# Dhia-naouali/dinov3-jax

Hardware: AMD Instinct MI355X
Metric: images/sec (whole node) ViT-L/16 DINOv3 pretrain 224px (higher is better)
Workload: dtype bf16; 1 GPU; model=vit_large, global_batch=64, img_size=224, local_crops=8, parallelism=dp1

## Files before the change

dinov3_amd/ops/csrc/bindings.hip:

```cpp

#include <torch/extension.h>
#include <ATen/hip/HIPContext.h>
#include <hip/hip_runtime.h>
#include <hip/hip_bf16.h>

#include <vector>

#define CHECK_INPUT(x) \
  TORCH_CHECK(x.is_cuda() && x.is_contiguous(), #x " must be a contiguous HIP tensor")

template <typename T>
void launch_layernorm_fwd(const T*, const T*, const T*, T*, float*, float*, long, int,
                          float, hipStream_t);
template <typename T>
void launch_layernorm_bwd(const T*, const T*, const T*, const float*, const float*, T*,
                          float*, float*, long, int, hipStream_t);
template <typename T>
void launch_rmsnorm_fwd(const T*, const T*, T*, float*, long, int, float, hipStream_t);
template <typename T>
void launch_rmsnorm_bwd(const T*, const T*, const T*, const float*, T*, float*, long, int,
                        hipStream_t);
template <typename T>
void launch_l2norm_fwd(const T*, T*, float*, long, int, float, hipStream_t);
template <typename T>
void launch_l2norm_bwd(const T*, const T*, const float*, T*, long, int, float, hipStream_t);
template <typename T>
void launch_bias_gelu_fwd(const T*, const T*, T*, long, int, hipStream_t);
template <typename T>
void launch_bias_gelu_bwd(const T*, const T*, const T*, T*, float*, long, int, hipStream_t);
template <typename T>
void launch_ls_axpy_fwd(const T*, const T*, const T*, T*, long, int, hipStream_t);
template <typename T>
void launch_ls_axpy_bwd(const T*, const T*, const T*, T*, float*, long, int, hipStream_t);
template <typename T>
void launch_ls_axpy_bias_fwd(const T*, const T*, const T*, const T*, T*, long, int,
                             hipStream_t);
template <typename T>
void launch_ls_axpy_bias_bwd(const T*, const T*, const T*, const T*, T*, float*, float*,
                             long, int, hipStream_t);
template <typename T>
void launch_ls_scatter_add(T*, const long*, const T*, const T*, const T*, const float*,
                           long, int, hipStream_t);
template <typename T>
void launch_ls_scatter_bwd(const T*, const long*, const T*, const T*, const T*,
                           const float*, T*, float*, float*, long, int, hipStream_t);
template <typename T>
void launch_row_gather(const T*, const long*, T*, long, int, hipStream_t);
template <typename T>
void launch_row_scatter_add(T*, const long*, const T*, const float*, long, int,
                            hipStream_t);
template <typename T>
void launch_row_gather_scaled(const T*, const long*, const float*, T*, long, int,
                              hipStream_t);
template <typename T>
void launch_swiglu_fwd(const T*, T*, long, int, hipStream_t);
template <typename T>
void launch_swiglu_bwd(const T*, const T*, T*, long, int, hipStream_t);
template <typename T>
void launch_rope_fwd(const T*, const float*, const float*, T*, long, int, int, int,
                     hipStream_t);
void launch_dino_ce_fwd(const __hip_bfloat16*, const float*, float*, float*, float*, int,
                        int, int, long, float, bool, hipStream_t);
void launch_dino_ce_bwd(const __hip_bfloat16*, const float*, const float*, const float*,
                        const float*, __hip_bfloat16*, int, int, int, long, float, bool,
                        hipStream_t);
void launch_ibot_ce_fwd(const __hip_bfloat16*, const float*, const float*, float*, float*,
                        float*, int, long, float, hipStream_t);
void launch_ibot_ce_bwd(const __hip_bfloat16*, const float*, const float*, const float*,
                        const float*, const float*, __hip_bfloat16*, int, long, float,
                        hipStream_t);
void launch_sinkhorn_exp(const __hip_bfloat16*, float*, float*, long, float, hipStream_t);
void launch_sinkhorn_fact_colsum(const __hip_bfloat16*, const float*, float*, int, long,
                                 float, hipStream_t);
void launch_sinkhorn_fact_rowsum(const __hip_bfloat16*, const float*, float*, int, long,
                                 float, hipStream_t);
void launch_ibot_ce_fact_fwd(const __hip_bfloat16*, const __hip_bfloat16*, const float*,
                             const float*, const float*, float*, float*, float*, int,
                             long, float, float, hipStream_t);
void launch_ibot_ce_fact_bwd(const __hip_bfloat16*, const __hip_bfloat16*, const float*,
                             const float*, const float*, const float*, const float*,
                             const float*, __hip_bfloat16*, int, long, float, float,
                             hipStream_t);
void launch_dino_ce_fact_fwd(const __hip_bfloat16*, const __hip_bfloat16*, const float*,
                             const float*, float*, float*, float*, int, int, int, long,
                             float, float, bool, hipStream_t);
void launch_dino_ce_fact_bwd(const __hip_bfloat16*, const __hip_bfloat16*, const float*,
                             const float*, const float*, const float*, const float*,
                             __hip_bfloat16*, int, int, int, long, float, float, bool,
                             hipStream_t);
void launch_sinkhorn_colsum(const float*, float*, int, long, const float*, hipStream_t);
void launch_sinkhorn_div_row(float*, const float*, int, long, float, const float*, bool,
                             hipStream_t);
void launch_fmha_rope_fwd(const __hip_bfloat16*, const float*, const float*,
                          __hip_bfloat16*, float*, int, int, int, int, int, float,
                          hipStream_t);
void launch_fmha_rope_bwd_pre(const __hip_bfloat16*, const __hip_bfloat16*, float*, int,
                              int, int, int, hipStream_t);
void launch_fmha_rope_bwd_dq(const __hip_bfloat16*, const __hip_bfloat16*, const float*,
                             const float*, const float*, const float*, __hip_bfloat16*,
                             int, int, int, int, int, float, hipStream_t);
void launch_fmha_rope_bwd_dkv(const __hip_bfloat16*, const __hip_bfloat16*, const float*,
                              const float*, const float*, const float*, __hip_bfloat16*,
                              int, int, int, int, int, float, hipStream_t);
void launch_patch_embed_fwd(const __hip_bfloat16*, const __hip_bfloat16*,
                            const __hip_bfloat16*, __hip_bfloat16*, int, int, int, int,
                            int, int, hipStream_t);
void launch_probe_mfma(const __hip_bfloat16*, const __hip_bfloat16*, float*, hipStream_t);
void launch_fmha_fwd(const __hip_bfloat16*, const __hip_bfloat16*, const __hip_bfloat16*,
                     __hip_bfloat16*, float*, int, int, int, float, hipStream_t);
void launch_fmha_bwd_pre(const __hip_bfloat16*, const __hip_bfloat16*, float*, long, int,
                         hipStream_t);
void launch_fmha_bwd_dq(const __hip_bfloat16*, const __hip_bfloat16*, const __hip_bfloat16*,
                        const __hip_bfloat16*, const float*, const float*, __hip_bfloat16*,
                        int, int, int, float, hipStream_t);
void launch_fmha_bwd_dkv(const __hip_bfloat16*, const __hip_bfloat16*,
                         const __hip_bfloat16*, const __hip_bfloat16*, const float*,
                         const float*, __hip_bfloat16*, __hip_bfloat16*, int, int, int,
                         float, hipStream_t);
template <typename T>
void launch_multi_tensor_ema(T* const*, const T* const*, const long*, const int*,
                             const long*, int, float, hipStream_t);
template <typename T>
void launch_multi_tensor_adamw(T* const*, const T* const*, float* const*, float* const*,
                               float* const*, const long*, const int*, const long*, int,
                               float, float, float, float, float, float, float, float,
                               bool, hipStream_t);
template <typename T>
void launch_multi_tensor_l2norm_sq(const T* const*, const long*, const int*, const long*,
                                   int, float*, hipStream_t);
template <typename T, typename GT>
void launch_multi_tensor_adamw_planned(T* const*, const GT* const*, float* const*,
                                       float* const*, float* const*, const long*,
                                       const int*, const long*, int, const float*,
                                       const float*, const float*, const int*,
                                       const float*, float, float, float, float, float,
                                       float, float, float, bool, hipStream_t);
template <typename T>
void launch_multi_tensor_l2norm_planned(const T* const*, const long*, const int*,
                                        const long*, int, const int*, float*,
                                        hipStream_t);

namespace {

hipStream_t current_stream() { return at::hip::getCurrentHIPStream().stream(); }

#define DISPATCH_FLOAT_BF16(TYPE, NAME, ...)                                   \
  [&] {                                                                        \
    if (TYPE == at::ScalarType::Float) {                                       \
      using scalar_t = float;                                                  \
      return __VA_ARGS__();                                                    \
    } else if (TYPE == at::ScalarType::BFloat16) {                             \
      using scalar_t = __hip_bfloat16;                                         \
      return __VA_ARGS__();                                                    \
    } else {                                                                   \
      TORCH_CHECK(false, NAME ": unsupported dtype ", TYPE);                   \
    }                                                                          \
  }()


std::vector<torch::Tensor> layernorm_fwd(torch::Tensor x, torch::Tensor w, torch::Tensor b,
                                         double eps) {
  CHECK_INPUT(x);
  const int D = x.size(-1);
  const long rows = x.numel() / D;
  auto y = torch::empty_like(x);
  auto mean = torch::empty({rows}, x.options().dtype(torch::kFloat));
  auto rstd = torch::empty({rows}, x.options().dtype(torch::kFloat));
  DISPATCH_FLOAT_BF16(x.scalar_type(), "layernorm_fwd", [&] {
    launch_layernorm_fwd<scalar_t>(
        (const scalar_t*)x.data_ptr(), (const scalar_t*)w.data_ptr(),
        (const scalar_t*)b.data_ptr(), (scalar_t*)y.data_ptr(),
        mean.data_ptr<float>(), rstd.data_ptr<float>(), rows, D, (float)eps,
        current_stream());
  });
  return {y, mean, rstd};
}

std::vector<torch::Tensor> layernorm_bwd(torch::Tensor dy, torch::Tensor x, torch::Tensor w,
                                         torch::Tensor mean, torch::Tensor rstd) {
  CHECK_INPUT(dy);
  CHECK_INPUT(x);
  const int D = x.size(-1);
  const long rows = x.numel() / D;
  auto dx = torch::empty_like(x);
  auto dw = torch::zeros({32, D}, x.options().dtype(torch::kFloat));
  auto db = torch::zeros({32, D}, x.options().dtype(torch::kFloat));
  DISPATCH_FLOAT_BF16(x.scalar_type(), "layernorm_bwd", [&] {
    launch_layernorm_bwd<scalar_t>(
        (const scalar_t*)dy.data_ptr(), (const scalar_t*)x.data_ptr(),
        (const scalar_t*)w.data_ptr(), mean.data_ptr<float>(), rstd.data_ptr<float>(),
        (scalar_t*)dx.data_ptr(), dw.data_ptr<float>(), db.data_ptr<float>(), rows, D,
        current_stream());
  });
  return {dx, dw.sum(0).to(x.scalar_type()), db.sum(0).to(x.scalar_type())};
}

std::vector<torch::Tensor> rmsnorm_fwd(torch::Tensor x, torch::Tensor w, double eps) {
  CHECK_INPUT(x);
  const int D = x.size(-1);
  const long rows = x.numel() / D;
  auto y = torch::empty_like(x);
  auto rstd = torch::empty({rows}, x.options().dtype(torch::kFloat));
  DISPATCH_FLOAT_BF16(x.scalar_type(), "rmsnorm_fwd", [&] {
    launch_rmsnorm_fwd<scalar_t>((const scalar_t*)x.data_ptr(), (const scalar_t*)w.data_ptr(),
                                 (scalar_t*)y.data_ptr(), rstd.data_ptr<float>(), rows, D,
                                 (float)eps, current_stream());
  });
  return {y, rstd};
}

std::vector<torch::Tensor> rmsnorm_bwd(torch::Tensor dy, torch::Tensor x, torch::Tensor w,
                                       torch::Tensor rstd) {
  CHECK_INPUT(dy);
  const int D = x.size(-1);
  const long rows = x.numel() / D;
  auto dx = torch::empty_like(x);
  auto dw = torch::zeros({D}, x.options().dtype(torch::kFloat));
  DISPATCH_FLOAT_BF16(x.scalar_type(), "rmsnorm_bwd", [&] {
    launch_rmsnorm_bwd<scalar_t>((const scalar_t*)dy.data_ptr(), (const scalar_t*)x.data_ptr(),
                                 (const scalar_t*)w.data_ptr(), rstd.data_ptr<float>(),
                                 (scalar_t*)dx.data_ptr(), dw.data_ptr<float>(), rows, D,
                                 current_stream());
  });
  return {dx, dw.to(x.scalar_type())};
}

std::vector<torch::Tensor> l2norm_fwd(torch::Tensor x, double eps) {
  CHECK_INPUT(x);
  const int D = x.size(-1);
  const long rows = x.numel() / D;
  auto y = torch::empty_like(x);
  auto s = torch::empty({rows}, x.options().dtype(torch::kFloat));
  DISPATCH_FLOAT_BF16(x.scalar_type(), "l2norm_fwd", [&] {
    launch_l2norm_fwd<scalar_t>((const scalar_t*)x.data_ptr(), (scalar_t*)y.data_ptr(),
                                s.data_ptr<float>(), rows, D, (float)eps, current_stream());
  });
  return {y, s};
}

torch::Tensor l2norm_bwd(torch::Tensor dy, torch::Tensor y, torch::Tensor s, double eps) {
  CHECK_INPUT(dy);
  const int D = y.size(-1);
  const long rows = y.numel() / D;
  auto dx = torch::empty_like(y);
  DISPATCH_FLOAT_BF16(y.scalar_type(), "l2norm_bwd", [&] {
    launch_l2norm_bwd<scalar_t>((const scalar_t*)dy.data_ptr(), (const scalar_t*)y.data_ptr(),
                                s.data_ptr<float>(), (scalar_t*)dx.data_ptr(), rows, D,
                                (float)eps, current_stream());
  });
  return dx;
}


torch::Tensor bias_gelu_fwd(torch::Tensor x, torch::Tensor bias) {
  CHECK_INPUT(x);
  const int H = x.size(-1);
  TORCH_CHECK(H % 8 == 0, "bias_gelu: H must be a multiple of 8");
  const long rows = x.numel() / H;
  auto y = torch::empty_like(x);
  DISPATCH_FLOAT_BF16(x.scalar_type(), "bias_gelu_fwd", [&] {
    launch_bias_gelu_fwd<scalar_t>((const scalar_t*)x.data_ptr(),
                                   (const scalar_t*)bias.data_ptr(), (scalar_t*)y.data_ptr(),
                                   rows, H, current_stream());
  });
  return y;
}

std::vector<torch::Tensor> bias_gelu_bwd(torch::Tensor dy, torch::Tensor x,
                                         torch::Tensor bias) {
  CHECK_INPUT(dy);
  const int H = x.size(-1);
  const long rows = x.numel() / H;
  auto dx = torch::empty_like(x);
  auto dbias = torch::zeros({32, H}, x.options().dtype(torch::kFloat));
  DISPATCH_FLOAT_BF16(x.scalar_type(), "bias_gelu_bwd", [&] {
    launch_bias_gelu_bwd<scalar_t>((const scalar_t*)dy.data_ptr(),
                                   (const scalar_t*)x.data_ptr(),
                                   (const scalar_t*)bias.data_ptr(), (scalar_t*)dx.data_ptr(),
                                   dbias.data_ptr<float>(), rows, H, current_stream());
  });
  return {dx, dbias.sum(0).to(x.scalar_type())};
}

torch::Tensor ls_axpy_fwd(torch::Tensor x, torch::Tensor res, torch::Tensor gamma) {
  CHECK_INPUT(x);
  CHECK_INPUT(res);
  const int D = x.size(-1);
  TORCH_CHECK(D % 8 == 0, "ls_axpy: D must be a multiple of 8");
  const long rows = x.numel() / D;
  auto out = torch::empty_like(x);
  DISPATCH_FLOAT_BF16(x.scalar_type(), "ls_axpy_fwd", [&] {
    launch_ls_axpy_fwd<scalar_t>((const scalar_t*)x.data_ptr(),
                                 (const scalar_t*)res.data_ptr(),
                                 (const scalar_t*)gamma.data_ptr(),
                                 (scalar_t*)out.data_ptr(), rows, D, current_stream());
  });
  return out;
}

torch::Tensor ls_axpy_bias_fwd(torch::Tensor x, torch::Tensor res, torch::Tensor gamma,
                               torch::Tensor bias) {
  CHECK_INPUT(x);
  CHECK_INPUT(res);
  const int D = x.size(-1);
  TORCH_CHECK(D % 8 == 0, "ls_axpy_bias: D must be a multiple of 8");
  const long rows = x.numel() / D;
  auto out = torch::empty_like(x);
  DISPATCH_FLOAT_BF16(x.scalar_type(), "ls_axpy_bias_fwd", [&] {
    launch_ls_axpy_bias_fwd<scalar_t>(
        (const scalar_t*)x.data_ptr(), (const scalar_t*)res.data_ptr(),
        (const scalar_t*)gamma.data_ptr(), (const scalar_t*)bias.data_ptr(),
        (scalar_t*)out.data_ptr(), rows, D, current_stream());
  });
  return out;
}

std::vector<torch::Tensor> ls_axpy_bwd(torch::Tensor dout, torch::Tensor res,
                                       torch::Tensor gamma) {
  CHECK_INPUT(dout);
  const int D = dout.size(-1);
  const long rows = dout.numel() / D;
  auto dres = torch::empty_like(dout);
  auto dgamma = torch::zeros({32, D}, dout.options().dtype(torch::kFloat));
  DISPATCH_FLOAT_BF16(dout.scalar_type(), "ls_axpy_bwd", [&] {
    launch_ls_axpy_bwd<scalar_t>((const scalar_t*)dout.data_ptr(),
                                 (const scalar_t*)res.data_ptr(),
                                 (const scalar_t*)gamma.data_ptr(),
                                 (scalar_t*)dres.data_ptr(), dgamma.data_ptr<float>(),
                                 rows, D, current_stream());
  });
  return {dres, dgamma.sum(0).to(dout.scalar_type())};
}

std::vector<torch::Tensor> ls_axpy_bias_bwd(torch::Tensor dout, torch::Tensor res,
                                            torch::Tensor gamma, torch::Tensor bias) {
  CHECK_INPUT(dout);
  const int D = dout.size(-1);
  const long rows = dout.numel() / D;
  auto dres = torch::empty_like(dout);
  auto fopt = dout.options().dtype(torch::kFloat);
  auto dgamma = torch::zeros({32, D}, fopt);
  auto dbias = torch::zeros({32, D}, fopt);
  DISPATCH_FLOAT_BF16(dout.scalar_type(), "ls_axpy_bias_bwd", [&] {
    launch_ls_axpy_bias_bwd<scalar_t>(
        (const scalar_t*)dout.data_ptr(), (const scalar_t*)res.data_ptr(),
        (const scalar_t*)gamma.data_ptr(), (const scalar_t*)bias.data_ptr(),
        (scalar_t*)dres.data_ptr(), dgamma.data_ptr<float>(), dbias.data_ptr<float>(),
        rows, D, current_stream());
  });
  return {dres, dgamma.sum(0).to(dout.scalar_type()), dbias.sum(0).to(dout.scalar_type())};
}

torch::Tensor row_gather(torch::Tensor src, torch::Tensor idx) {
  CHECK_INPUT(src);
  const int D = src.size(-1);
  TORCH_CHECK(D % 8 == 0, "row ops need D % 8 == 0");
  const long M = idx.numel();
  auto out = torch::empty({M, D}, src.options());
  DISPATCH_FLOAT_BF16(src.scalar_type(), "row_gather", [&] {
    launch_row_gather<scalar_t>((const scalar_t*)src.data_ptr(), idx.data_ptr<long>(),
                                (scalar_t*)out.data_ptr(), M, D, current_stream());
  });
  return out;
}

void row_scatter_add_(torch::Tensor dst, torch::Tensor idx, torch::Tensor src,
                      torch::Tensor scale) {
  CHECK_INPUT(dst);
  CHECK_INPUT(src);
  const int D = dst.size(-1);
  const long M = idx.numel();
  const float* sp = (scale.defined() && scale.numel() > 0) ? scale.data_ptr<float>() : nullptr;
  DISPATCH_FLOAT_BF16(dst.scalar_type(), "row_scatter_add", [&] {
    launch_row_scatter_add<scalar_t>((scalar_t*)dst.data_ptr(), idx.data_ptr<long>(),
                                     (const scalar_t*)src.data_ptr(), sp, M, D,
                                     current_stream());
  });
}

torch::Tensor row_gather_scaled(torch::Tensor src, torch::Tensor idx, torch::Tensor scale) {
  CHECK_INPUT(src);
  const int D = src.size(-1);
  const long M = idx.numel();
  auto out = torch::empty({M, D}, src.options());
  const float* sp = (scale.defined() && scale.numel() > 0) ? scale.data_ptr<float>() : nullptr;
  DISPATCH_FLOAT_BF16(src.scalar_type(), "row_gather_scaled", [&] {
    launch_row_gather_scaled<scalar_t>((const scalar_t*)src.data_ptr(),
                                       idx.data_ptr<long>(), sp, (scalar_t*)out.data_ptr(),
                                       M, D, current_stream());
  });
  return out;
}

void ls_scatter_add_(torch::Tensor dst, torch::Tensor idx, torch::Tensor src,
                     torch::Tensor gamma, torch::Tensor bias, torch::Tensor scale) {
  CHECK_INPUT(dst);
  CHECK_INPUT(src);
  const int D = dst.size(-1);
  TORCH_CHECK(D % 8 == 0, "ls_scatter: D must be a multiple of 8");
  const long M = idx.numel();
  DISPATCH_FLOAT_BF16(dst.scalar_type(), "ls_scatter_add_", [&] {
    launch_ls_scatter_add<scalar_t>(
        (scalar_t*)dst.data_ptr(), idx.data_ptr<long>(), (const scalar_t*)src.data_ptr(),
        gamma.defined() ? (const scalar_t*)gamma.data_ptr() : nullptr,
        bias.defined() ? (const scalar_t*)bias.data_ptr() : nullptr,
        scale.defined() && scale.numel() > 0 ? scale.data_ptr<float>() : nullptr, M, D,
        current_stream());
  });
}

std::vector<torch::Tensor> ls_scatter_bwd(torch::Tensor dy, torch::Tensor idx,
                                          torch::Tensor src, torch::Tensor gamma,
                                          torch::Tensor bias, torch::Tensor scale) {
  CHECK_INPUT(dy);
  CHECK_INPUT(src);
  const int D = dy.size(-1);
  const long M = idx.numel();
  auto dres = torch::empty_like(src);
  auto fopt = dy.options().dtype(torch::kFloat);
  auto dgamma = gamma.defined() ? torch::zeros({32, D}, fopt) : torch::Tensor();
  auto dbias = bias.defined() ? torch::zeros({32, D}, fopt) : torch::Tensor();
  DISPATCH_FLOAT_BF16(dy.scalar_type(), "ls_scatter_bwd", [&] {
    launch_ls_scatter_bwd<scalar_t>(
        (const scalar_t*)dy.data_ptr(), idx.data_ptr<long>(),
        (const scalar_t*)src.data_ptr(),
        gamma.defined() ? (const scalar_t*)gamma.data_ptr() : nullptr,
        bias.defined() ? (const scalar_t*)bias.data_ptr() : nullptr,
        scale.defined() && scale.numel() > 0 ? scale.data_ptr<float>() : nullptr,
        (scalar_t*)dres.data_ptr(),
        dgamma.defined() ? dgamma.data_ptr<float>() : nullptr,
        dbias.defined() ? dbias.data_ptr<float>() : nullptr, M, D, current_stream());
  });
  return {dres, dgamma.defined() ? dgamma.sum(0).to(dy.scalar_type()) : dgamma,
          dbias.defined() ? dbias.sum(0).to(dy.scalar_type()) : dbias};
}

torch::Tensor swiglu_fwd(torch::Tensor x12) {
  CHECK_INPUT(x12);
  const int H2 = x12.size(-1);
  const int H = H2 / 2;
  const long rows = x12.numel() / H2;
  auto sizes = x12.sizes().vec();
  sizes.back() = H;
  auto y = torch::empty(sizes, x12.options());
  DISPATCH_FLOAT_BF16(x12.scalar_type(), "swiglu_fwd", [&] {
    launch_swiglu_fwd<scalar_t>((const scalar_t*)x12.data_ptr(), (scalar_t*)y.data_ptr(),
                                rows, H, current_stream());
  });
  return y;
}

torch::Tensor swiglu_bwd(torch::Tensor dy, torch::Tensor x12) {
  CHECK_INPUT(dy);
  const int H2 = x12.size(-1);
  const int H = H2 / 2;
  const long rows = x12.numel() / H2;
  auto dx12 = torch::empty_like(x12);
  DISPATCH_FLOAT_BF16(x12.scalar_type(), "swiglu_bwd", [&] {
    launch_swiglu_bwd<scalar_t>((const scalar_t*)dy.data_ptr(),
                                (const scalar_t*)x12.data_ptr(), (scalar_t*)dx12.data_ptr(),
                                rows, H, current_stream());
  });
  return dx12;
}

torch::Tensor rope_fwd(torch::Tensor x, torch::Tensor sin_t, torch::Tensor cos_t,
                       int64_t prefix) {
  CHECK_INPUT(x);
  TORCH_CHECK(x.dim() == 4, "rope_fwd expects [B, H, N, hd]");
  TORCH_CHECK(sin_t.scalar_type() == at::ScalarType::Float, "rope tables must be fp32");
  const long BH = x.size(0) * x.size(1);
  const int N = x.size(2);
  const int hd = x.size(3);
  const int P = N - (int)prefix;
  TORCH_CHECK(sin_t.size(0) == P && sin_t.size(1) == hd, "rope table shape mismatch");
  auto y = torch::empty_like(x);
  DISPATCH_FLOAT_BF16(x.scalar_type(), "rope_fwd", [&] {
    launch_rope_fwd<scalar_t>((const scalar_t*)x.data_ptr(), sin_t.data_ptr<float>(),
                              cos_t.data_ptr<float>(), (scalar_t*)y.data_ptr(), BH, N, P, hd,
                              current_stream());
  });
  return y;
}


std::vector<torch::Tensor> dino_ce_fwd(torch::Tensor x, torch::Tensor t, double temp,
                                       bool ignore_diag) {
  CHECK_INPUT(x);
  CHECK_INPUT(t);
  TORCH_CHECK(x.dim() == 3 && t.dim() == 3, "dino_ce expects [S,B,K] and [T,B,K]");
  TORCH_CHECK(x.scalar_type() == at::ScalarType::BFloat16);
  TORCH_CHECK(t.scalar_type() == at::ScalarType::Float);
  const int S = x.size(0), B = x.size(1);
  const int T = t.size(0);
  const long K = x.size(2);
  auto lse = torch::empty({S * B}, x.options().dtype(torch::kFloat));
  auto st = torch::empty({S * B}, x.options().dtype(torch::kFloat));
  auto loss = torch::zeros({}, x.options().dtype(torch::kFloat));
  launch_dino_ce_fwd((const __hip_bfloat16*)x.data_ptr(), t.data_ptr<float>(),
                     lse.data_ptr<float>(), st.data_ptr<float>(), loss.data_ptr<float>(),
                     S, T, B, K, (float)(1.0 / temp), ignore_diag, current_stream());
  return {loss, lse, st};
}

torch::Tensor dino_ce_bwd(torch::Tensor g, torch::Tensor x, torch::Tensor t,
                          torch::Tensor lse, torch::Tensor st, double temp,
                          bool ignore_diag) {
  const int S = x.size(0), B = x.size(1);
  const int T = t.size(0);
  const long K = x.size(2);
  auto dx = torch::empty_like(x);
  launch_dino_ce_bwd((const __hip_bfloat16*)x.data_ptr(), t.data_ptr<float>(),
                     lse.data_ptr<float>(), st.data_ptr<float>(), g.data_ptr<float>(),
                     (__hip_bfloat16*)dx.data_ptr(), S, T, B, K, (float)(1.0 / temp),
                     ignore_diag, current_stream());
  return dx;
}

std::vector<torch::Tensor> ibot_ce_fwd(torch::Tensor x, torch::Tensor t, torch::Tensor w,
                                       double temp) {
  CHECK_INPUT(x);
  CHECK_INPUT(t);
  const int M = x.size(0);
  const long K = x.size(1);
  auto lse = torch::empty({M}, x.options().dtype(torch::kFloat));
  auto st = torch::empty({M}, x.options().dtype(torch::kFloat));
  auto loss = torch::zeros({}, x.options().dtype(torch::kFloat));
  launch_ibot_ce_fwd((const __hip_bfloat16*)x.data_ptr(), t.data_ptr<float>(),
                     w.data_ptr<float>(), lse.data_ptr<float>(), st.data_ptr<float>(),
                     loss.data_ptr<float>(), M, K, (float)(1.0 / temp), current_stream());
  return {loss, lse, st};
}

torch::Tensor ibot_ce_bwd(torch::Tensor g, torch::Tensor x, torch::Tensor t,
                          torch::Tensor w, torch::Tensor lse, torch::Tensor st,
                          double temp) {
  const int M = x.size(0);
  const long K = x.size(1);
  auto dx = torch::empty_like(x);
  launch_ibot_ce_bwd((const __hip_bfloat16*)x.data_ptr(), t.data_ptr<float>(),
                     w.data_ptr<float>(), lse.data_ptr<float>(), st.data_ptr<float>(),
                     g.data_ptr<float>(), (__hip_bfloat16*)dx.data_ptr(), M, K,
                     (float)(1.0 / temp), current_stream());
  return dx;
}

torch::Tensor sinkhorn_fact_colsum(torch::Tensor x, torch::Tensor u, double temp) {
  CHECK_INPUT(x);
  const int M = x.size(0);
  const long K = x.size(1);
  auto A = torch::empty({K}, x.options().dtype(torch::kFloat));
  const float* up = (u.defined() && u.numel() > 0) ? u.data_ptr<float>() : nullptr;
  launch_sinkhorn_fact_colsum((const __hip_bfloat16*)x.data_ptr(), up,
                              A.data_ptr<float>(), M, K, (float)(1.0 / temp),
                              current_stream());
  return A;
}

torch::Tensor sinkhorn_fact_rowsum(torch::Tensor x, torch::Tensor v, double temp) {
  CHECK_INPUT(x);
  const int M = x.size(0);
  const long K = x.size(1);
  auto u = torch::empty({M}, x.options().dtype(torch::kFloat));
  launch_sinkhorn_fact_rowsum((const __hip_bfloat16*)x.data_ptr(), v.data_ptr<float>(),
                              u.data_ptr<float>(), M, K, (float)(1.0 / temp),
                              current_stream());
  return u;
}

std::vector<torch::Tensor> ibot_ce_fact_fwd(torch::Tensor x, torch::Tensor xt,
                                            torch::Tensor u, torch::Tensor v,
                                            torch::Tensor w, double temp, double tt) {
  CHECK_INPUT(x);
  CHECK_INPUT(xt);
  const int M = x.size(0);
  const long K = x.size(1);
  auto lse = torch::empty({M}, x.options().dtype(torch::kFloat));
  auto st = torch::empty({M}, x.options().dtype(torch::kFloat));
  auto loss = torch::zeros({}, x.options().dtype(torch::kFloat));
  launch_ibot_ce_fact_fwd((const __hip_bfloat16*)x.data_ptr(),
                          (const __hip_bfloat16*)xt.data_ptr(), u.data_ptr<float>(),
                          v.data_ptr<float>(), w.data_ptr<float>(), lse.data_ptr<float>(),
                          st.data_ptr<float>(), loss.data_ptr<float>(), M, K,
                          (float)(1.0 / temp), (float)(1.0 / tt), current_stream());
  return {loss, lse, st};
}

torch::Tensor ibot_ce_fact_bwd(torch::Tensor g, torch::Tensor x, torch::Tensor xt,
                               torch::Tensor u, torch::Tensor v, torch::Tensor w,
                               torch::Tensor lse, torch::Tensor st, double temp,
                               double tt) {
  const int M = x.size(0);
  const long K = x.size(1);
  auto dx = torch::empty_like(x);
  launch_ibot_ce_fact_bwd((const __hip_bfloat16*)x.data_ptr(),
                          (const __hip_bfloat16*)xt.data_ptr(), u.data_ptr<float>(),
                          v.data_ptr<float>(), w.data_ptr<float>(), lse.data_ptr<float>(),
                          st.data_ptr<float>(), g.data_ptr<float>(),
                          (__hip_bfloat16*)dx.data_ptr(), M, K, (float)(1.0 / temp),
                          (float)(1.0 / tt), current_stream());
  return dx;
}

std::vector<torch::Tensor> dino_ce_fact_fwd(torch::Tensor x, torch::Tensor xt,
                                            torch::Tensor u, torch::Tensor v, double temp,
                                            double tt, bool ignore_diag) {
  CHECK_INPUT(x);
  CHECK_INPUT(xt);
  const int S = x.size(0), B = x.size(1);
  const int T = xt.size(0);
  const long K = x.size(2);
  auto lse = torch::empty({S * B}, x.options().dtype(torch::kFloat));
  auto st = torch::empty({S * B}, x.options().dtype(torch::kFloat));
  auto loss = torch::zeros({}, x.options().dtype(torch::kFloat));
  launch_dino_ce_fact_fwd((const __hip_bfloat16*)x.data_ptr(),
                          (const __hip_bfloat16*)xt.data_ptr(), u.data_ptr<float>(),
                          v.data_ptr<float>(), lse.data_ptr<float>(), st.data_ptr<float>(),
                          loss.data_ptr<float>(), S, T, B, K, (float)(1.0 / temp),
                          (float)(1.0 / tt), ignore_diag, current_stream());
  return {loss, lse, st};
}

torch::Tensor dino_ce_fact_bwd(torch::Tensor g, torch::Tensor x, torch::Tensor xt,
                               torch::Tensor u, torch::Tensor v, torch::Tensor lse,
                               torch::Tensor st, double temp, double tt,
                               bool ignore_diag) {
  const int S = x.size(0), B = x.size(1);
  const int T = xt.size(0);
  const long K = x.size(2);
  auto dx = torch::empty_like(x);
  launch_dino_ce_fact_bwd((const __hip_bfloat16*)x.data_ptr(),
                          (const __hip_bfloat16*)xt.data_ptr(), u.data_ptr<float>(),
                          v.data_ptr<float>(), lse.data_ptr<float>(), st.data_ptr<float>(),
                          g.data_ptr<float>(), (__hip_bfloat16*)dx.data_ptr(), S, T, B, K,
                          (float)(1.0 / temp), (float)(1.0 / tt), ignore_diag,
                          current_stream());
  return dx;
}

std::vector<torch::Tensor> sinkhorn_exp(torch::Tensor x, double temp) {
  CHECK_INPUT(x);
  auto Q = torch::empty(x.sizes(), x.options().dtype(torch::kFloat));
  auto total = torch::zeros({}, x.options().dtype(torch::kFloat));
  launch_sinkhorn_exp((const __hip_bfloat16*)x.data_ptr(), Q.data_ptr<float>(),
                      total.data_ptr<float>(), x.numel(), (float)(1.0 / temp),
                      current_stream());
  return {Q, total};
}

torch::Tensor sinkhorn_colsum(torch::Tensor Q, torch::Tensor divisor) {
  const int M = Q.size(0);
  const long K = Q.size(1);
  auto out = torch::empty({K}, Q.options());
  launch_sinkhorn_colsum(Q.data_ptr<float>(), out.data_ptr<float>(), M, K,
                         divisor.data_ptr<float>(), current_stream());
  return out;
}

void sinkhorn_div_row(torch::Tensor Q, torch::Tensor col, double k_div, torch::Tensor B,
                      bool scale_back) {
  const int M = Q.size(0);
  const long K = Q.size(1);
  launch_sinkhorn_div_row(Q.data_ptr<float>(), col.data_ptr<float>(), M, K, (float)k_div,
                          B.data_ptr<float>(), scale_back, current_stream());
}


torch::Tensor probe_mfma(torch::Tensor A, torch::Tensor B) {
  CHECK_INPUT(A);
  CHECK_INPUT(B);
  TORCH_CHECK(A.scalar_type() == at::ScalarType::BFloat16);
  auto C = torch::empty({32, 32}, A.options().dtype(torch::kFloat));
  launch_probe_mfma((const __hip_bfloat16*)A.data_ptr(), (const __hip_bfloat16*)B.data_ptr(),
                    C.data_ptr<float>(), current_stream());
  return C;
}

std::vector<torch::Tensor> fmha_fwd(torch::Tensor q, torch::Tensor k, torch::Tensor v) {
  CHECK_INPUT(q);
  CHECK_INPUT(k);
  CHECK_INPUT(v);
  TORCH_CHECK(q.scalar_type() == at::ScalarType::BFloat16, "fmha: bf16 only");
  TORCH_CHECK(q.dim() == 4, "fmha expects [B, H, N, hd]");
  const int B = q.size(0), H = q.size(1), N = q.size(2), HD = q.size(3);
  TORCH_CHECK(HD == 64 || HD == 128, "fmha: head_dim must be 64 or 128, got ", HD);
  auto o = torch::empty_like(q);
  auto lse = torch::empty({B, H, N}, q.options().dtype(torch::kFloat));
  const float scale = 1.0f / std::sqrt((float)HD);
  launch_fmha_fwd((const __hip_bfloat16*)q.data_ptr(), (const __hip_bfloat16*)k.data_ptr(),
                  (const __hip_bfloat16*)v.data_ptr(), (__hip_bfloat16*)o.data_ptr(),
                  lse.data_ptr<float>(), B * H, N, HD, scale, current_stream());
  return {o, lse};
}

std::vector<torch::Tensor> fmha_bwd(torch::Tensor dout, torch::Tensor q, torch::Tensor k,
                                    torch::Tensor v, torch::Tensor o, torch::Tensor lse) {
  CHECK_INPUT(dout);
  const int B = q.size(0), H = q.size(1), N = q.size(2), HD = q.size(3);
  const float scale = 1.0f / std::sqrt((float)HD);
  auto D = torch::empty({B, H, N}, q.options().dtype(torch::kFloat));
  auto dq = torch::empty_like(q);
  auto dk = torch::empty_like(k);
  auto dv = torch::empty_like(v);
  auto stream = current_stream();
  launch_fmha_bwd_pre((const __hip_bfloat16*)dout.data_ptr(),
                      (const __hip_bfloat16*)o.data_ptr(), D.data_ptr<float>(),
                      (long)B * H * N, HD, stream);
  launch_fmha_bwd_dq((const __hip_bfloat16*)q.data_ptr(), (const __hip_bfloat16*)k.data_ptr(),
                     (const __hip_bfloat16*)v.data_ptr(),
                     (const __hip_bfloat16*)dout.data_ptr(), lse.data_ptr<float>(),
                     D.data_ptr<float>(), (__hip_bfloat16*)dq.data_ptr(), B * H, N, HD,
                     scale, stream);
  launch_fmha_bwd_dkv((const __hip_bfloat16*)q.data_ptr(), (const __hip_bfloat16*)k.data_ptr(),
                      (const __hip_bfloat16*)v.data_ptr(),
                      (const __hip_bfloat16*)dout.data_ptr(), lse.data_ptr<float>(),
                      D.data_ptr<float>(), (__hip_bfloat16*)dk.data_ptr(),
                      (__hip_bfloat16*)dv.data_ptr(), B * H, N, HD, scale, stream);
  return {dq, dk, dv};
}


torch::Tensor patch_embed_fwd(torch::Tensor x, torch::Tensor w, torch::Tensor bias,
                              int64_t patch) {
  CHECK_INPUT(x);
  CHECK_INPUT(w);
  TORCH_CHECK(x.dim() == 4 && x.scalar_type() == at::ScalarType::BFloat16);
  const int B = x.size(0), C = x.size(1), H = x.size(2), W = x.size(3);
  const int D = w.size(0);
  TORCH_CHECK(C == 3, "patch_embed_fwd kernel supports C=3 (any patch size)");
  TORCH_CHECK(H % patch == 0 && W % patch == 0, "H/W must be multiples of patch");
  const long rows = (long)B * (H / patch) * (W / patch);
  auto out = torch::empty({(long)B, rows / B, (long)D}, x.options());
  launch_patch_embed_fwd((const __hip_bfloat16*)x.data_ptr(),
                         (const __hip_bfloat16*)w.data_ptr(),
                         (const __hip_bfloat16*)bias.data_ptr(),
                         (__hip_bfloat16*)out.data_ptr(), B, C, H, W, (int)patch, D,
                         current_stream());
  return out;
}


std::vector<torch::Tensor> fmha_rope_fwd_out(torch::Tensor qkv, torch::Tensor sin_t,
                                             torch::Tensor cos_t, int64_t prefix,
                                             torch::Tensor out_o) {
  CHECK_INPUT(qkv);
  TORCH_CHECK(qkv.dim() == 5 && qkv.size(2) == 3, "qkv must be [B, N, 3, H, hd]");
  TORCH_CHECK(qkv.scalar_type() == at::ScalarType::BFloat16);
  const int B = qkv.size(0), N = qkv.size(1), H = qkv.size(3), HD = qkv.size(4);
  TORCH_CHECK(HD == 64 || HD == 128, "head_dim must be 64 or 128");
  const bool has_rope = sin_t.defined() && sin_t.numel() > 0;
  const int P = has_rope ? (int)sin_t.size(0) : N - (int)prefix;
  if (has_rope) {
    TORCH_CHECK(sin_t.scalar_type() == at::ScalarType::Float && sin_t.is_contiguous());
    TORCH_CHECK(P == N - prefix, "rope table rows must equal N - prefix");
  }
  torch::Tensor o = out_o.defined() && out_o.numel() > 0 ? out_o
                                                        : torch::empty({B, N, H, HD}, qkv.options());
  TORCH_CHECK(o.is_contiguous() && o.numel() == (long)B * N * H * HD);
  auto lse = torch::empty({B, H, N}, qkv.options().dtype(torch::kFloat));
  const float scale = 1.0f / std::sqrt((float)HD);
  launch_fmha_rope_fwd((const __hip_bfloat16*)qkv.data_ptr(),
                       has_rope ? sin_t.data_ptr<float>() : nullptr,
                       has_rope ? cos_t.data_ptr<float>() : nullptr,
                       (__hip_bfloat16*)o.data_ptr(), lse.data_ptr<float>(), B, H, N, P,
                       HD, scale, current_stream());
  return {o, lse};
}

torch::Tensor fmha_rope_bwd_out(torch::Tensor dout, torch::Tensor qkv, torch::Tensor o,
                                torch::Tensor lse, torch::Tensor sin_t,
                                torch::Tensor cos_t, int64_t prefix,
                                torch::Tensor out_dqkv) {
  CHECK_INPUT(dout);
  const int B = qkv.size(0), N = qkv.size(1), H = qkv.size(3), HD = qkv.size(4);
  const bool has_rope = sin_t.defined() && sin_t.numel() > 0;
  const int P = N - (int)prefix;
  const float scale = 1.0f / std::sqrt((float)HD);
  auto D = torch::empty({B, H, N}, qkv.options().dtype(torch::kFloat));
  torch::Tensor dqkv = out_dqkv.defined() && out_dqkv.numel() > 0 ? out_dqkv
                                                                  : torch::empty_like(qkv);
  auto stream = current_stream();
  launch_fmha_rope_bwd_pre((const __hip_bfloat16*)dout.data_ptr(),
                           (const __hip_bfloat16*)o.data_ptr(), D.data_ptr<float>(), B, H,
                           N, HD, stream);
  launch_fmha_rope_bwd_dq((const __hip_bfloat16*)qkv.data_ptr(),
                          (const __hip_bfloat16*)dout.data_ptr(),
                          has_rope ? sin_t.data_ptr<float>() : nullptr,
                          has_rope ? cos_t.data_ptr<float>() : nullptr,
                          lse.data_ptr<float>(), D.data_ptr<float>(),
                          (__hip_bfloat16*)dqkv.data_ptr(), B, H, N, P, HD, scale, stream);
  launch_fmha_rope_bwd_dkv((const __hip_bfloat16*)qkv.data_ptr(),
                           (const __hip_bfloat16*)dout.data_ptr(),
                           has_rope ? sin_t.data_ptr<float>() : nullptr,
                           has_rope ? cos_t.data_ptr<float>() : nullptr,
                           lse.data_ptr<float>(), D.data_ptr<float>(),
                           (__hip_bfloat16*)dqkv.data_ptr(), B, H, N, P, HD, scale,
                           stream);
  return dqkv;
}



void multi_tensor_ema_planned(torch::Tensor ptrs, torch::Tensor sizes, torch::Tensor ct,
                              torch::Tensor co, int64_t n_tensors, double m,
                              bool is_bf16) {
  const int n_chunks = (int)ct.numel();
  long* pp = ptrs.data_ptr<long>();
  if (is_bf16) {
    launch_multi_tensor_ema<__hip_bfloat16>(
        (__hip_bfloat16* const*)pp, (const __hip_bfloat16* const*)(pp + n_tensors),
        sizes.data_ptr<long>(), ct.data_ptr<int>(), co.data_ptr<long>(), n_chunks,
        (float)m, current_stream());
  } else {
    launch_multi_tensor_ema<float>(
        (float* const*)pp, (const float* const*)(pp + n_tensors), sizes.data_ptr<long>(),
        ct.data_ptr<int>(), co.data_ptr<long>(), n_chunks, (float)m, current_stream());
  }
}

void multi_tensor_adamw_planned(torch::Tensor ptrs, torch::Tensor sizes, torch::Tensor ct,
                                torch::Tensor co, int64_t n_tensors, torch::Tensor lr_mult,
                                torch::Tensor wd_mult, torch::Tensor is_last,
                                torch::Tensor sub_id, torch::Tensor clip, double lr,
                                double last_lr, double wd, double beta1, double beta2,
                                double eps, double bc1, double bc2, bool has_master,
                                bool is_bf16, bool grad_is_f32) {
  const int n_chunks = (int)ct.numel();
  long* pp = ptrs.data_ptr<long>();
  const long n = n_tensors;
  if (is_bf16 && grad_is_f32) {
    launch_multi_tensor_adamw_planned<__hip_bfloat16, float>(
        (__hip_bfloat16* const*)pp, (const float* const*)(pp + n),
        (float* const*)(pp + 2 * n), (float* const*)(pp + 3 * n),
        has_master ? (float* const*)(pp + 4 * n) : nullptr, sizes.data_ptr<long>(),
        ct.data_ptr<int>(), co.data_ptr<long>(), n_chunks, lr_mult.data_ptr<float>(),
        wd_mult.data_ptr<float>(), is_last.data_ptr<float>(), sub_id.data_ptr<int>(),
        clip.data_ptr<float>(), (float)lr, (float)last_lr, (float)wd, (float)beta1,
        (float)beta2, (float)eps, (float)bc1, (float)bc2, has_master, current_stream());
  } else if (is_bf16) {
    launch_multi_tensor_adamw_planned<__hip_bfloat16, __hip_bfloat16>(
        (__hip_bfloat16* const*)pp, (const __hip_bfloat16* const*)(pp + n),
        (float* const*)(pp + 2 * n), (float* const*)(pp + 3 * n),
        has_master ? (float* const*)(pp + 4 * n) : nullptr, sizes.data_ptr<long>(),
        ct.data_ptr<int>(), co.data_ptr<long>(), n_chunks, lr_mult.data_ptr<float>(),
        wd_mult.data_ptr<float>(), is_last.data_ptr<float>(), sub_id.data_ptr<int>(),
        clip.data_ptr<float>(), (float)lr, (float)last_lr, (float)wd, (float)beta1,
        (float)beta2, (float)eps, (float)bc1, (float)bc2, has_master, current_stream());
  } else {
    launch_multi_tensor_adamw_planned<float, float>(
        (float* const*)pp, (const float* const*)(pp + n), (float* const*)(pp + 2 * n),
        (float* const*)(pp + 3 * n), has_master ? (float* const*)(pp + 4 * n) : nullptr,
        sizes.data_ptr<long>(), ct.data_ptr<int>(), co.data_ptr<long>(), n_chunks,
        lr_mult.data_ptr<float>(), wd_mult.data_ptr<float>(), is_last.data_ptr<float>(),
        sub_id.data_ptr<int>(), clip.data_ptr<float>(), (float)lr, (float)last_lr,
        (float)wd, (float)beta1, (float)beta2, (float)eps, (float)bc1, (float)bc2,
        has_master, current_stream());
  }
}

torch::Tensor multi_tensor_l2norm_planned(torch::Tensor ptrs, torch::Tensor sizes,
                                          torch::Tensor ct, torch::Tensor co,
                                          torch::Tensor sub_id, int64_t n_submodels,
                                          bool is_bf16) {
  const int n_chunks = (int)ct.numel();
  auto out = torch::zeros({n_submodels}, torch::dtype(torch::kFloat).device(ptrs.device()));
  long* pp = ptrs.data_ptr<long>();
  if (is_bf16) {
    launch_multi_tensor_l2norm_planned<__hip_bfloat16>(
        (const __hip_bfloat16* const*)pp, sizes.data_ptr<long>(), ct.data_ptr<int>(),
        co.data_ptr<long>(), n_chunks, sub_id.data_ptr<int>(), out.data_ptr<float>(),
        current_stream());
  } else {
    launch_multi_tensor_l2norm_planned<float>(
        (const float* const*)pp, sizes.data_ptr<long>(), ct.data_ptr<int>(),
        co.data_ptr<long>(), n_chunks, sub_id.data_ptr<int>(), out.data_ptr<float>(),
        current_stream());
  }
  return out;
}


struct MTTables {
  torch::Tensor device_buf;
  long* sizes;
  int* chunk_tensor;
  long* chunk_offset;
  long* ptr_arrays;
  int n_chunks;
  int n_tensors;
};

constexpr long kMTChunk = 65536;

MTTables build_tables(const std::vector<std::vector<torch::Tensor>>& lists,
                      torch::Device device) {
  const int n_tensors = (int)lists[0].size();
  const int n_lists = (int)lists.size();
  std::vector<long> sizes(n_tensors);
  std::vector<int> chunk_tensor;
  std::vector<long> chunk_offset;
  for (int t = 0; t < n_tensors; ++t) {
    sizes[t] = lists[0][t].numel();
    for (long off = 0; off < sizes[t]; off += kMTChunk) {
      chunk_tensor.push_back(t);
      chunk_offset.push_back(off);
    }
  }
  const int n_chunks = (int)chunk_tensor.size();
  const long total = n_tensors + n_chunks + n_chunks + (long)n_lists * n_tensors;
  auto host = torch::empty({total}, torch::dtype(torch::kLong).pinned_memory(true));
  long* hp = host.data_ptr<long>();
  long* p_sizes = hp;
  long* p_ct = hp + n_tensors;
  long* p_co = p_ct + n_chunks;
  long* p_ptr = p_co + n_chunks;
  for (int t = 0; t < n_tensors; ++t) p_sizes[t] = sizes[t];
  for (int c = 0; c < n_chunks; ++c) {
    p_ct[c] = chunk_tensor[c];
    p_co[c] = chunk_offset[c];
  }
  for (int l = 0; l < n_lists; ++l)
    for (int t = 0; t < n_tensors; ++t)
      p_ptr[(long)l * n_tensors + t] = (long)(uintptr_t)lists[l][t].data_ptr();
  auto dev = host.to(device, true);
  MTTables out;
  out.device_buf = dev;
  long* dp = dev.data_ptr<long>();
  out.sizes = dp;
  out.chunk_tensor = nullptr;
  out.chunk_offset = dp + n_tensors + n_chunks;
  out.ptr_arrays = dp + n_tensors + 2 * (long)n_chunks;
  out.n_chunks = n_chunks;
  out.n_tensors = n_tensors;
  return out;
}

torch::Tensor build_chunk_tensor_i32(const std::vector<long>& sizes, torch::Device device,
                                     int* n_chunks_out) {
  std::vector<int> ct;
  for (int t = 0; t < (int)sizes.size(); ++t)
    for (long off = 0; off < sizes[t]; off += kMTChunk) ct.push_back(t);
  *n_chunks_out = (int)ct.size();
  auto host = torch::from_blob(ct.data(), {(long)ct.size()}, torch::kInt).clone();
  return host.to(device);
}

void multi_tensor_ema(std::vector<torch::Tensor> t_list, std::vector<torch::Tensor> s_list,
                      double m) {
  TORCH_CHECK(!t_list.empty() && t_list.size() == s_list.size());
  auto device = t_list[0].device();
  auto tables = build_tables({t_list, s_list}, device);
  std::vector<long> sizes(tables.n_tensors);
  for (int t = 0; t < tables.n_tensors; ++t) sizes[t] = t_list[t].numel();
  int n_chunks;
  auto ct32 = build_chunk_tensor_i32(sizes, device, &n_chunks);
  auto stream = current_stream();
  DISPATCH_FLOAT_BF16(t_list[0].scalar_type(), "multi_tensor_ema", [&] {
    launch_multi_tensor_ema<scalar_t>(
        (scalar_t* const*)(tables.ptr_arrays),
        (const scalar_t* const*)(tables.ptr_arrays + tables.n_tensors),
        tables.sizes, ct32.data_ptr<int>(), tables.chunk_offset, n_chunks, (float)m, stream);
  });
}

void multi_tensor_adamw(std::vector<torch::Tensor> p, std::vector<torch::Tensor> g,
                        std::vector<torch::Tensor> m, std::vector<torch::Tensor> v,
                        std::vector<torch::Tensor> w, double lr, double beta1, double beta2,
                        double eps, double weight_decay, double bc1, double bc2,
                        double grad_scale) {
  TORCH_CHECK(!p.empty());
  const bool has_master = !w.empty();
  auto device = p[0].device();
  std::vector<std::vector<torch::Tensor>> lists = {p, g, m, v};
  if (has_master) lists.push_back(w);
  auto tables = build_tables(lists, device);
  std::vector<long> sizes(tables.n_tensors);
  for (int t = 0; t < tables.n_tensors; ++t) sizes[t] = p[t].numel();
  int n_chunks;
  auto ct32 = build_chunk_tensor_i32(sizes, device, &n_chunks);
  auto stream = current_stream();
  const int nt = tables.n_tensors;
  DISPATCH_FLOAT_BF16(p[0].scalar_type(), "multi_tensor_adamw", [&] {
    launch_multi_tensor_adamw<scalar_t>(
        (scalar_t* const*)(tables.ptr_arrays),
        (const scalar_t* const*)(tables.ptr_arrays + nt),
        (float* const*)(tables.ptr_arrays + 2L * nt),
        (float* const*)(tables.ptr_arrays + 3L * nt),
        has_master ? (float* const*)(tables.ptr_arrays + 4L * nt) : nullptr,
        tables.sizes, ct32.data_ptr<int>(), tables.chunk_offset, n_chunks, (float)lr,
        (float)beta1, (float)beta2, (float)eps, (float)weight_decay, (float)bc1, (float)bc2,
        (float)grad_scale, has_master, stream);
  });
}

torch::Tensor multi_tensor_l2norm_sq(std::vector<torch::Tensor> g) {
  TORCH_CHECK(!g.empty());
  auto device = g[0].device();
  auto tables = build_tables({g}, device);
  std::vector<long> sizes(tables.n_tensors);
  for (int t = 0; t < tables.n_tensors; ++t) sizes[t] = g[t].numel();
  int n_chunks;
  auto ct32 = build_chunk_tensor_i32(sizes, device, &n_chunks);
  auto out = torch::zeros({}, torch::dtype(torch::kFloat).device(device));
  DISPATCH_FLOAT_BF16(g[0].scalar_type(), "multi_tensor_l2norm_sq", [&] {
    launch_multi_tensor_l2norm_sq<scalar_t>(
        (const scalar_t* const*)(tables.ptr_arrays), tables.sizes, ct32.data_ptr<int>(),
        tables.chunk_offset, n_chunks, out.data_ptr<float>(), current_stream());
  });
  return out;
}

}

std::vector<torch::Tensor> blaslt_gemm_bias_gelu_fwd(torch::Tensor x, torch::Tensor w,
                                                     torch::Tensor bias);
std::vector<torch::Tensor> blaslt_gemm_dgelu_bgrad(torch::Tensor dy, torch::Tensor w2,
                                                   torch::Tensor pre);
torch::Tensor blaslt_gemm_bias(torch::Tensor x, torch::Tensor w, torch::Tensor bias);
int64_t blaslt_probe_epilogue(int64_t epi, int64_t aux_type, int64_t bias_type,
                              int64_t m, int64_t n, int64_t k);

PYBIND11_MODULE(TORCH_EXTENSION_NAME, mod) {
  mod.def("blaslt_gemm_bias_gelu_fwd", &blaslt_gemm_bias_gelu_fwd);
  mod.def("blaslt_gemm_dgelu_bgrad", &blaslt_gemm_dgelu_bgrad);
  mod.def("blaslt_gemm_bias", &blaslt_gemm_bias);
  mod.def("blaslt_probe_epilogue", &blaslt_probe_epilogue);
  mod.def("layernorm_fwd", &layernorm_fwd);
  mod.def("layernorm_bwd", &layernorm_bwd);
  mod.def("rmsnorm_fwd", &rmsnorm_fwd);
  mod.def("rmsnorm_bwd", &rmsnorm_bwd);
  mod.def("l2norm_fwd", &l2norm_fwd);
  mod.def("l2norm_bwd", &l2norm_bwd);
  mod.def("bias_gelu_fwd", &bias_gelu_fwd);
  mod.def("bias_gelu_bwd", &bias_gelu_bwd);
  mod.def("row_gather", &row_gather);
  mod.def("row_scatter_add_", &row_scatter_add_);
  mod.def("row_gather_scaled", &row_gather_scaled);
  mod.def("ls_axpy_fwd", &ls_axpy_fwd);
  mod.def("ls_axpy_bias_fwd", &ls_axpy_bias_fwd);
  mod.def("ls_axpy_bias_bwd", &ls_axpy_bias_bwd);
  mod.def("ls_scatter_add_", &ls_scatter_add_);
  mod.def("ls_scatter_bwd", &ls_scatter_bwd);
  mod.def("ls_axpy_bwd", &ls_axpy_bwd);
  mod.def("swiglu_fwd", &swiglu_fwd);
  mod.def("swiglu_bwd", &swiglu_bwd);
  mod.def("rope_fwd", &rope_fwd);
  mod.def("probe_mfma", &probe_mfma);
  mod.def("patch_embed_fwd", &patch_embed_fwd);
  mod.def("dino_ce_fwd", &dino_ce_fwd);
  mod.def("dino_ce_bwd", &dino_ce_bwd);
  mod.def("ibot_ce_fwd", &ibot_ce_fwd);
  mod.def("ibot_ce_bwd", &ibot_ce_bwd);
  mod.def("sinkhorn_exp", &sinkhorn_exp);
  mod.def("sinkhorn_fact_colsum", &sinkhorn_fact_colsum);
  mod.def("sinkhorn_fact_rowsum", &sinkhorn_fact_rowsum);
  mod.def("ibot_ce_fact_fwd", &ibot_ce_fact_fwd);
  mod.def("ibot_ce_fact_bwd", &ibot_ce_fact_bwd);
  mod.def("dino_ce_fact_fwd", &dino_ce_fact_fwd);
  mod.def("dino_ce_fact_bwd", &dino_ce_fact_bwd);
  mod.def("sinkhorn_colsum", &sinkhorn_colsum);
  mod.def("sinkhorn_div_row", &sinkhorn_div_row);
  mod.def("fmha_fwd", &fmha_fwd);
  mod.def("fmha_rope_fwd", [](torch::Tensor qkv, torch::Tensor sin_t, torch::Tensor cos_t,
                              int64_t prefix) {
    return fmha_rope_fwd_out(qkv, sin_t, cos_t, prefix, torch::Tensor());
  });
  mod.def("fmha_rope_fwd_out", &fmha_rope_fwd_out);
  mod.def("fmha_rope_bwd", [](torch::Tensor dout, torch::Tensor qkv, torch::Tensor o,
                              torch::Tensor lse, torch::Tensor sin_t, torch::Tensor cos_t,
                              int64_t prefix) {
    return fmha_rope_bwd_out(dout, qkv, o, lse, sin_t, cos_t, prefix, torch::Tensor());
  });
  mod.def("fmha_rope_bwd_out", &fmha_rope_bwd_out);
  mod.def("fmha_bwd", &fmha_bwd);
  mod.def("multi_tensor_ema", &multi_tensor_ema);
  mod.def("multi_tensor_ema_planned", &multi_tensor_ema_planned);
  mod.def("multi_tensor_adamw_planned", &multi_tensor_adamw_planned);
  mod.def("multi_tensor_l2norm_planned", &multi_tensor_l2norm_planned);
  mod.def("multi_tensor_adamw", &multi_tensor_adamw);
  mod.def("multi_tensor_l2norm_sq", &multi_tensor_l2norm_sq);
}
```

dinov3_amd/ops/csrc/common.h:

```cpp
#pragma once

#include <hip/hip_runtime.h>
#include <hip/hip_bf16.h>
#include <hip/hip_fp16.h>

#define WAVE_SIZE 64
#define DEV_INLINE __device__ __forceinline__

typedef __attribute__((ext_vector_type(8))) short short8_t;
typedef __attribute__((ext_vector_type(4))) float float4_t;

DEV_INLINE float bf16_to_f32(short u) {
  union { float f; unsigned int i; } v;
  v.i = ((unsigned int)(unsigned short)u) << 16;
  return v.f;
}

DEV_INLINE short f32_to_bf16(float f) {
  union { float f; unsigned int i; } v;
  v.f = f;
  unsigned int rounding_bias = 0x7FFF + ((v.i >> 16) & 1);
  return (short)((v.i + rounding_bias) >> 16);
}

template <typename T> struct ScalarOps;

template <> struct ScalarOps<float> {
  DEV_INLINE static float load(const float* p) { return *p; }
  DEV_INLINE static void store(float* p, float v) { *p = v; }
};

template <> struct ScalarOps<__hip_bfloat16> {
  DEV_INLINE static float load(const __hip_bfloat16* p) {
    return bf16_to_f32(*reinterpret_cast<const short*>(p));
  }
  DEV_INLINE static void store(__hip_bfloat16* p, float v) {
    *reinterpret_cast<short*>(p) = f32_to_bf16(v);
  }
};

template <> struct ScalarOps<_Float16> {
  DEV_INLINE static float load(const _Float16* p) { return (float)(*p); }
  DEV_INLINE static void store(_Float16* p, float v) { *p = (_Float16)v; }
};

template <typename T> struct Vec8 {
  DEV_INLINE static void load(T* dst, const T* src) {
    reinterpret_cast<float4_t*>(dst)[0] = reinterpret_cast<const float4_t*>(src)[0];
    reinterpret_cast<float4_t*>(dst)[1] = reinterpret_cast<const float4_t*>(src)[1];
  }
  DEV_INLINE static void store(T* dst, const T* src) {
    reinterpret_cast<float4_t*>(dst)[0] = reinterpret_cast<const float4_t*>(src)[0];
    reinterpret_cast<float4_t*>(dst)[1] = reinterpret_cast<const float4_t*>(src)[1];
  }
};

template <> struct Vec8<__hip_bfloat16> {
  DEV_INLINE static void load(__hip_bfloat16* dst, const __hip_bfloat16* src) {
    *reinterpret_cast<float4_t*>(dst) = *reinterpret_cast<const float4_t*>(src);
  }
  DEV_INLINE static void store(__hip_bfloat16* dst, const __hip_bfloat16* src) {
    *reinterpret_cast<float4_t*>(dst) = *reinterpret_cast<const float4_t*>(src);
  }
};

DEV_INLINE float wave_reduce_sum(float v) {
#pragma unroll
  for (int off = WAVE_SIZE / 2; off > 0; off >>= 1) v += __shfl_down(v, off, WAVE_SIZE);
  return v;
}

DEV_INLINE float wave_reduce_max(float v) {
#pragma unroll
  for (int off = WAVE_SIZE / 2; off > 0; off >>= 1) v = fmaxf(v, __shfl_down(v, off, WAVE_SIZE));
  return v;
}

DEV_INLINE float block_reduce_sum(float v, float* lds) {
  const int lane = threadIdx.x & (WAVE_SIZE - 1);
  const int wid = threadIdx.x / WAVE_SIZE;
  v = wave_reduce_sum(v);
  if (lane == 0) lds[wid] = v;
  __syncthreads();
  const int nw = (blockDim.x + WAVE_SIZE - 1) / WAVE_SIZE;
  v = (threadIdx.x < nw) ? lds[threadIdx.x] : 0.0f;
  if (wid == 0) v = wave_reduce_sum(v);
  if (threadIdx.x == 0) lds[0] = v;
  __syncthreads();
  return lds[0];
}

DEV_INLINE float block_reduce_max(float v, float* lds) {
  const int lane = threadIdx.x & (WAVE_SIZE - 1);
  const int wid = threadIdx.x / WAVE_SIZE;
  v = wave_reduce_max(v);
  if (lane == 0) lds[wid] = v;
  __syncthreads();
  const int nw = (blockDim.x + WAVE_SIZE - 1) / WAVE_SIZE;
  v = (threadIdx.x < nw) ? lds[threadIdx.x] : -INFINITY;
  if (wid == 0) v = wave_reduce_max(v);
  if (threadIdx.x == 0) lds[0] = v;
  __syncthreads();
  return lds[0];
}

#define HIP_CHECK_LAUNCH()                                                    \
  do {                                                                        \
    hipError_t e = hipGetLastError();                                         \
    if (e != hipSuccess) {                                                    \
      printf("HIP launch error: %s at %s:%d\n", hipGetErrorString(e),         \
             __FILE__, __LINE__);                                             \
    }                                                                         \
  } while (0)
```

dinov3_amd/ops/csrc/elementwise.hip:

```cpp

#include "common.h"

#define EW_BLOCK 256
#define EW_SHADOWS 32

DEV_INLINE float fast_tanh(float y) {
  return 1.0f - 2.0f / (1.0f + __expf(2.0f * y));
}

DEV_INLINE float gelu_tanh(float x) {
  const float k0 = 0.7978845608028654f;
  const float k1 = 0.044715f;
  float inner = k0 * (x + k1 * x * x * x);
  return 0.5f * x * (1.0f + fast_tanh(inner));
}

DEV_INLINE float gelu_tanh_grad(float x) {
  const float k0 = 0.7978845608028654f;
  const float k1 = 0.044715f;
  float x2 = x * x;
  float inner = k0 * (x + k1 * x * x2);
  float t = fast_tanh(inner);
  float sech2 = 1.0f - t * t;
  return 0.5f * (1.0f + t) + 0.5f * x * sech2 * k0 * (1.0f + 3.0f * k1 * x2);
}


template <typename T>
__global__ void bias_gelu_fwd_kernel(const T* __restrict__ x, const T* __restrict__ bias,
                                     T* __restrict__ y, long rows, int H) {
  const long total8 = rows * (long)(H / 8);
  for (long idx = blockIdx.x * (long)blockDim.x + threadIdx.x; idx < total8;
       idx += (long)gridDim.x * blockDim.x) {
    const int col8 = (int)(idx % (H / 8)) * 8;
    const T* xp = x + idx * 8;
    T* yp = y + idx * 8;
    T xb[8], bb[8], yb[8];
    Vec8<T>::load(xb, xp);
    Vec8<T>::load(bb, bias + col8);
#pragma unroll
    for (int e = 0; e < 8; ++e) {
      float v = ScalarOps<T>::load(xb + e) + ScalarOps<T>::load(bb + e);
      ScalarOps<T>::store(yb + e, gelu_tanh(v));
    }
    Vec8<T>::store(yp, yb);
  }
}

template <typename T, int RR_ILP = 4>
__global__ void bias_gelu_bwd_kernel(const T* __restrict__ dy, const T* __restrict__ x,
                                     const T* __restrict__ bias, T* __restrict__ dx,
                                     float* __restrict__ dbias, long rows, int H) {
  const int col8 = (blockIdx.y * blockDim.x + threadIdx.x) * 8;
  if (col8 >= H) return;
  T bb[8];
  Vec8<T>::load(bb, bias + col8);
  float db[8] = {0.f, 0.f, 0.f, 0.f, 0.f, 0.f, 0.f, 0.f};
  long row = blockIdx.x * (long)RR_ILP;
  const long rstep = (long)gridDim.x * RR_ILP;
  for (; row + RR_ILP - 1 < rows; row += rstep) {
    T xb[RR_ILP][8], gb[RR_ILP][8], ob[RR_ILP][8];
#pragma unroll
    for (int rr = 0; rr < RR_ILP; ++rr) {
      const long off = (row + rr) * (long)H + col8;
      Vec8<T>::load(xb[rr], x + off);
      Vec8<T>::load(gb[rr], dy + off);
    }
#pragma unroll
    for (int rr = 0; rr < RR_ILP; ++rr) {
#pragma unroll
      for (int e = 0; e < 8; ++e) {
        float v = ScalarOps<T>::load(xb[rr] + e) + ScalarOps<T>::load(bb + e);
        float g = ScalarOps<T>::load(gb[rr] + e) * gelu_tanh_grad(v);
        ScalarOps<T>::store(ob[rr] + e, g);
        db[e] += g;
      }
      Vec8<T>::store(dx + (row + rr) * (long)H + col8, ob[rr]);
    }
  }
  for (; row < rows; ++row) {
    const long off = row * (long)H + col8;
    T xb[8], gb[8], ob[8];
    Vec8<T>::load(xb, x + off);
    Vec8<T>::load(gb, dy + off);
#pragma unroll
    for (int e = 0; e < 8; ++e) {
      float v = ScalarOps<T>::load(xb + e) + ScalarOps<T>::load(bb + e);
      float g = ScalarOps<T>::load(gb + e) * gelu_tanh_grad(v);
      ScalarOps<T>::store(ob + e, g);
      db[e] += g;
    }
    Vec8<T>::store(dx + off, ob);
  }
  float* dbias_s = dbias + (long)(blockIdx.x & (EW_SHADOWS - 1)) * H;
#pragma unroll
  for (int e = 0; e < 8; ++e) atomicAdd(dbias_s + col8 + e, db[e]);
}

template <typename T, int PASSES>
__global__ __launch_bounds__(256) void bias_gelu_bwd_rows_kernel(
    const T* __restrict__ dy, const T* __restrict__ x, const T* __restrict__ bias,
    T* __restrict__ dx, float* __restrict__ dbias, long rows, int H) {
  T bb[PASSES][8];
  float db[PASSES][8];
#pragma unroll
  for (int pss = 0; pss < PASSES; ++pss) {
    Vec8<T>::load(bb[pss], bias + (pss * 256 + threadIdx.x) * 8);
#pragma unroll
    for (int e = 0; e < 8; ++e) db[pss][e] = 0.f;
  }
  for (long row = blockIdx.x; row < rows; row += gridDim.x) {
    const long base = row * (long)H;
#pragma unroll
    for (int pss = 0; pss < PASSES; ++pss) {
      const long off = base + (pss * 256 + threadIdx.x) * 8;
      T xb[8], gb[8], ob[8];
      Vec8<T>::load(xb, x + off);
      Vec8<T>::load(gb, dy + off);
#pragma unroll
      for (int e = 0; e < 8; ++e) {
        const float v = ScalarOps<T>::load(xb + e) + ScalarOps<T>::load(bb[pss] + e);
        const float g = ScalarOps<T>::load(gb + e) * gelu_tanh_grad(v);
        ScalarOps<T>::store(ob + e, g);
        db[pss][e] += g;
      }
      Vec8<T>::store(dx + off, ob);
    }
  }
  float* dbias_s = dbias + (long)(blockIdx.x & (EW_SHADOWS - 1)) * H;
#pragma unroll
  for (int pss = 0; pss < PASSES; ++pss) {
    const int c8 = (pss * 256 + threadIdx.x) * 8;
#pragma unroll
    for (int e = 0; e < 8; ++e) atomicAdd(dbias_s + c8 + e, db[pss][e]);
  }
}


template <typename T>
__global__ void ls_axpy_fwd_kernel(const T* __restrict__ x, const T* __restrict__ res,
                                   const T* __restrict__ gamma, T* __restrict__ out,
                                   long rows, int D) {
  const long total8 = rows * (long)(D / 8);
  for (long idx = blockIdx.x * (long)blockDim.x + threadIdx.x; idx < total8;
       idx += (long)gridDim.x * blockDim.x) {
    const int col8 = (int)(idx % (D / 8)) * 8;
    T xb[8], rb[8], gb[8], ob[8];
    Vec8<T>::load(xb, x + idx * 8);
    Vec8<T>::load(rb, res + idx * 8);
    Vec8<T>::load(gb, gamma + col8);
#pragma unroll
    for (int e = 0; e < 8; ++e) {
      float v = ScalarOps<T>::load(xb + e) +
                ScalarOps<T>::load(gb + e) * ScalarOps<T>::load(rb + e);
      ScalarOps<T>::store(ob + e, v);
    }
    Vec8<T>::store(out + idx * 8, ob);
  }
}

template <typename T>
__global__ void ls_axpy_bwd_kernel(const T* __restrict__ dout, const T* __restrict__ res,
                                   const T* __restrict__ gamma, T* __restrict__ dres,
                                   float* __restrict__ dgamma, long rows, int D) {
  const int col8 = (blockIdx.y * blockDim.x + threadIdx.x) * 8;
  if (col8 >= D) return;
  T gb[8];
  Vec8<T>::load(gb, gamma + col8);
  float dg[8] = {0.f, 0.f, 0.f, 0.f, 0.f, 0.f, 0.f, 0.f};
  long row = blockIdx.x * 4L;
  const long rstep = (long)gridDim.x * 4;
  for (; row + 3 < rows; row += rstep) {
    T db[4][8], rb[4][8], ob[4][8];
#pragma unroll
    for (int rr = 0; rr < 4; ++rr) {
      Vec8<T>::load(db[rr], dout + (row + rr) * (long)D + col8);
      Vec8<T>::load(rb[rr], res + (row + rr) * (long)D + col8);
    }
#pragma unroll
    for (int rr = 0; rr < 4; ++rr) {
#pragma unroll
      for (int e = 0; e < 8; ++e) {
        const float g = ScalarOps<T>::load(db[rr] + e);
        dg[e] += g * ScalarOps<T>::load(rb[rr] + e);
        ScalarOps<T>::store(ob[rr] + e, g * ScalarOps<T>::load(gb + e));
      }
      Vec8<T>::store(dres + (row + rr) * (long)D + col8, ob[rr]);
    }
  }
  for (; row < rows; ++row) {
    const long off = row * (long)D + col8;
    T db[8], rb[8], ob[8];
    Vec8<T>::load(db, dout + off);
    Vec8<T>::load(rb, res + off);
#pragma unroll
    for (int e = 0; e < 8; ++e) {
      const float g = ScalarOps<T>::load(db + e);
      dg[e] += g * ScalarOps<T>::load(rb + e);
      ScalarOps<T>::store(ob + e, g * ScalarOps<T>::load(gb + e));
    }
    Vec8<T>::store(dres + off, ob);
  }
  float* dgamma_s = dgamma + (long)(blockIdx.x & (EW_SHADOWS - 1)) * D;
#pragma unroll
  for (int e = 0; e < 8; ++e) atomicAdd(dgamma_s + col8 + e, dg[e]);
}


template <typename T>
__global__ void ls_axpy_bias_fwd_kernel(const T* __restrict__ x, const T* __restrict__ res,
                                        const T* __restrict__ gamma,
                                        const T* __restrict__ bias, T* __restrict__ out,
                                        long rows, int D) {
  const long total8 = rows * (long)(D / 8);
  for (long idx = blockIdx.x * (long)blockDim.x + threadIdx.x; idx < total8;
       idx += (long)gridDim.x * blockDim.x) {
    const int col8 = (int)(idx % (D / 8)) * 8;
    T xb[8], rb[8], gb[8], bb[8], ob[8];
    Vec8<T>::load(xb, x + idx * 8);
    Vec8<T>::load(rb, res + idx * 8);
    Vec8<T>::load(gb, gamma + col8);
    Vec8<T>::load(bb, bias + col8);
#pragma unroll
    for (int e = 0; e < 8; ++e) {
      float v = ScalarOps<T>::load(xb + e) +
                ScalarOps<T>::load(gb + e) *
                    (ScalarOps<T>::load(rb + e) + ScalarOps<T>::load(bb + e));
      ScalarOps<T>::store(ob + e, v);
    }
    Vec8<T>::store(out + idx * 8, ob);
  }
}

template <typename T>
__global__ void ls_axpy_bias_bwd_kernel(const T* __restrict__ dout,
                                        const T* __restrict__ res,
                                        const T* __restrict__ gamma,
                                        const T* __restrict__ bias, T* __restrict__ dres,
                                        float* __restrict__ dgamma,
                                        float* __restrict__ dbias, long rows, int D) {
  const int col8 = (blockIdx.y * blockDim.x + threadIdx.x) * 8;
  if (col8 >= D) return;
  T gb[8], bb[8];
  Vec8<T>::load(gb, gamma + col8);
  Vec8<T>::load(bb, bias + col8);
  float dg[8] = {0.f, 0.f, 0.f, 0.f, 0.f, 0.f, 0.f, 0.f};
  float db_acc[8] = {0.f, 0.f, 0.f, 0.f, 0.f, 0.f, 0.f, 0.f};
  long row = blockIdx.x * 4L;
  const long rstep = (long)gridDim.x * 4;
  for (; row + 3 < rows; row += rstep) {
    T db[4][8], rb[4][8], ob[4][8];
#pragma unroll
    for (int rr = 0; rr < 4; ++rr) {
      Vec8<T>::load(db[rr], dout + (row + rr) * (long)D + col8);
      Vec8<T>::load(rb[rr], res + (row + rr) * (long)D + col8);
    }
#pragma unroll
    for (int rr = 0; rr < 4; ++rr) {
#pragma unroll
      for (int e = 0; e < 8; ++e) {
        const float g = ScalarOps<T>::load(db[rr] + e);
        const float gm = ScalarOps<T>::load(gb + e);
        dg[e] += g * (ScalarOps<T>::load(rb[rr] + e) + ScalarOps<T>::load(bb + e));
        db_acc[e] += g * gm;
        ScalarOps<T>::store(ob[rr] + e, g * gm);
      }
      Vec8<T>::store(dres + (row + rr) * (long)D + col8, ob[rr]);
    }
  }
  for (; row < rows; ++row) {
    const long off = row * (long)D + col8;
    T db[8], rb[8], ob[8];
    Vec8<T>::load(db, dout + off);
    Vec8<T>::load(rb, res + off);
#pragma unroll
    for (int e = 0; e < 8; ++e) {
      const float g = ScalarOps<T>::load(db + e);
      const float gm = ScalarOps<T>::load(gb + e);
      dg[e] += g * (ScalarOps<T>::load(rb + e) + ScalarOps<T>::load(bb + e));
      db_acc[e] += g * gm;
      ScalarOps<T>::store(ob + e, g * gm);
    }
    Vec8<T>::store(dres + off, ob);
  }
  const long sh = (long)(blockIdx.x & (EW_SHADOWS - 1)) * D;
#pragma unroll
  for (int e = 0; e < 8; ++e) {
    atomicAdd(dgamma + sh + col8 + e, dg[e]);
    atomicAdd(dbias + sh + col8 + e, db_acc[e]);
  }
}


template <typename T>
__global__ void ls_scatter_add_kernel(T* __restrict__ dst, const long* __restrict__ idx,
                                      const T* __restrict__ src,
                                      const T* __restrict__ gamma,
                                      const T* __restrict__ bias,
                                      const float* __restrict__ scale, long M, int D) {
  const int d8 = D / 8;
  long total = M * (long)d8;
  for (long i = blockIdx.x * (long)blockDim.x + threadIdx.x; i < total;
       i += (long)gridDim.x * blockDim.x) {
    const long r = i / d8;
    const int c8 = (int)(i % d8) * 8;
    const long drow = idx[r];
    const float s = scale != nullptr ? scale[r] : 1.0f;
    T sb[8], db[8], gb[8], bb[8];
    Vec8<T>::load(sb, src + r * (long)D + c8);
    Vec8<T>::load(db, dst + drow * (long)D + c8);
    if (gamma != nullptr) Vec8<T>::load(gb, gamma + c8);
    if (bias != nullptr) Vec8<T>::load(bb, bias + c8);
#pragma unroll
    for (int e = 0; e < 8; ++e) {
      const float g = gamma != nullptr ? ScalarOps<T>::load(gb + e) : 1.0f;
      const float bv = bias != nullptr ? ScalarOps<T>::load(bb + e) : 0.0f;
      ScalarOps<T>::store(
          db + e, ScalarOps<T>::load(db + e) + s * g * (ScalarOps<T>::load(sb + e) + bv));
    }
    Vec8<T>::store(dst + drow * (long)D + c8, db);
  }
}

template <typename T, int RR = 4>
__global__ void ls_scatter_bwd_kernel(const T* __restrict__ dy, const long* __restrict__ idx,
                                      const T* __restrict__ src,
                                      const T* __restrict__ gamma,
                                      const T* __restrict__ bias,
                                      const float* __restrict__ scale,
                                      T* __restrict__ dres, float* __restrict__ dgamma,
                                      float* __restrict__ dbias, long M, int D) {
  const int col8 = (blockIdx.y * blockDim.x + threadIdx.x) * 8;
  if (col8 >= D) return;
  T gb[8], bb[8];
  if (gamma != nullptr) Vec8<T>::load(gb, gamma + col8);
  if (bias != nullptr) Vec8<T>::load(bb, bias + col8);
  float dg[8] = {0.f, 0.f, 0.f, 0.f, 0.f, 0.f, 0.f, 0.f};
  float db_acc[8] = {0.f, 0.f, 0.f, 0.f, 0.f, 0.f, 0.f, 0.f};
  long r = blockIdx.x * (long)RR;
  const long rstep4 = (long)gridDim.x * RR;
  for (; r + RR - 1 < M; r += rstep4) {
    long srow[RR];
    float sc[RR];
    T dyb[RR][8], rb[RR][8], ob[RR][8];
#pragma unroll
    for (int rr = 0; rr < RR; ++rr) {
      srow[rr] = idx[r + rr];
      sc[rr] = scale != nullptr ? scale[r + rr] : 1.0f;
      Vec8<T>::load(dyb[rr], dy + srow[rr] * (long)D + col8);
      Vec8<T>::load(rb[rr], src + (r + rr) * (long)D + col8);
    }
#pragma unroll
    for (int rr = 0; rr < RR; ++rr) {
#pragma unroll
      for (int e = 0; e < 8; ++e) {
        const float gv = ScalarOps<T>::load(dyb[rr] + e) * sc[rr];
        const float gm = gamma != nullptr ? ScalarOps<T>::load(gb + e) : 1.0f;
        const float bv = bias != nullptr ? ScalarOps<T>::load(bb + e) : 0.0f;
        dg[e] += gv * (ScalarOps<T>::load(rb[rr] + e) + bv);
        db_acc[e] += gv * gm;
        ScalarOps<T>::store(ob[rr] + e, gv * gm);
      }
      Vec8<T>::store(dres + (r + rr) * (long)D + col8, ob[rr]);
    }
  }
  for (; r < M; ++r) {
    const long srow = idx[r];
    const float s = scale != nullptr ? scale[r] : 1.0f;
    T dyb[8], rb[8], ob[8];
    Vec8<T>::load(dyb, dy + srow * (long)D + col8);
    Vec8<T>::load(rb, src + r * (long)D + col8);
#pragma unroll
    for (int e = 0; e < 8; ++e) {
      const float gv = ScalarOps<T>::load(dyb + e) * s;
      const float gm = gamma != nullptr ? ScalarOps<T>::load(gb + e) : 1.0f;
      const float bv = bias != nullptr ? ScalarOps<T>::load(bb + e) : 0.0f;
      dg[e] += gv * (ScalarOps<T>::load(rb + e) + bv);
      db_acc[e] += gv * gm;
      ScalarOps<T>::store(ob + e, gv * gm);
    }
    Vec8<T>::store(dres + r * (long)D + col8, ob);
  }
  const long sh = (long)(blockIdx.x & (EW_SHADOWS - 1)) * D;
#pragma unroll
  for (int e = 0; e < 8; ++e) {
    if (dgamma != nullptr) atomicAdd(dgamma + sh + col8 + e, dg[e]);
    if (dbias != nullptr) atomicAdd(dbias + sh + col8 + e, db_acc[e]);
  }
}


template <typename T>
__global__ void swiglu_fwd_kernel(const T* __restrict__ x12, T* __restrict__ y,
                                  long rows, int H) {
  long total = rows * (long)H;
  for (long idx = blockIdx.x * (long)blockDim.x + threadIdx.x; idx < total;
       idx += (long)gridDim.x * blockDim.x) {
    long row = idx / H;
    int col = (int)(idx % H);
    const T* xr = x12 + row * (long)(2 * H);
    float x1 = ScalarOps<T>::load(xr + col);
    float x2 = ScalarOps<T>::load(xr + H + col);
    float sig = 1.0f / (1.0f + expf(-x1));
    ScalarOps<T>::store(y + idx, x1 * sig * x2);
  }
}

template <typename T>
__global__ void swiglu_bwd_kernel(const T* __restrict__ dy, const T* __restrict__ x12,
                                  T* __restrict__ dx12, long rows, int H) {
  long total = rows * (long)H;
  for (long idx = blockIdx.x * (long)blockDim.x + threadIdx.x; idx < total;
       idx += (long)gridDim.x * blockDim.x) {
    long row = idx / H;
    int col = (int)(idx % H);
    const T* xr = x12 + row * (long)(2 * H);
    T* dxr = dx12 + row * (long)(2 * H);
    float x1 = ScalarOps<T>::load(xr + col);
    float x2 = ScalarOps<T>::load(xr + H + col);
    float g = ScalarOps<T>::load(dy + idx);
    float sig = 1.0f / (1.0f + expf(-x1));
    float silu = x1 * sig;
    float dsilu = sig * (1.0f + x1 * (1.0f - sig));
    ScalarOps<T>::store(dxr + col, g * x2 * dsilu);
    ScalarOps<T>::store(dxr + H + col, g * silu);
  }
}


template <typename T>
__global__ void row_gather_kernel(const T* __restrict__ src, const long* __restrict__ idx,
                                  T* __restrict__ out, long M, int D) {
  const int d8 = D / 8;
  long total = M * (long)d8;
  for (long i = blockIdx.x * (long)blockDim.x + threadIdx.x; i < total;
       i += (long)gridDim.x * blockDim.x) {
    const long r = i / d8;
    const int c8 = (int)(i % d8) * 8;
    const long srow = idx[r];
    T buf[8];
    Vec8<T>::load(buf, src + srow * (long)D + c8);
    Vec8<T>::store(out + r * (long)D + c8, buf);
  }
}

template <typename T>
__global__ void row_scatter_add_kernel(T* __restrict__ dst, const long* __restrict__ idx,
                                       const T* __restrict__ src,
                                       const float* __restrict__ scale, long M, int D) {
  const int d8 = D / 8;
  long total = M * (long)d8;
  for (long i = blockIdx.x * (long)blockDim.x + threadIdx.x; i < total;
       i += (long)gridDim.x * blockDim.x) {
    const long r = i / d8;
    const int c8 = (int)(i % d8) * 8;
    const long drow = idx[r];
    const float s = scale != nullptr ? scale[r] : 1.0f;
    T sb[8], db[8];
    Vec8<T>::load(sb, src + r * (long)D + c8);
    Vec8<T>::load(db, dst + drow * (long)D + c8);
#pragma unroll
    for (int e = 0; e < 8; ++e) {
      ScalarOps<T>::store(db + e,
                          ScalarOps<T>::load(db + e) + s * ScalarOps<T>::load(sb + e));
    }
    Vec8<T>::store(dst + drow * (long)D + c8, db);
  }
}

template <typename T>
__global__ void row_gather_scaled_kernel(const T* __restrict__ src,
                                         const long* __restrict__ idx,
                                         const float* __restrict__ scale,
                                         T* __restrict__ out, long M, int D) {
  const int d8 = D / 8;
  long total = M * (long)d8;
  for (long i = blockIdx.x * (long)blockDim.x + threadIdx.x; i < total;
       i += (long)gridDim.x * blockDim.x) {
    const long r = i / d8;
    const int c8 = (int)(i % d8) * 8;
    const long srow = idx[r];
    const float s = scale != nullptr ? scale[r] : 1.0f;
    T buf[8];
    Vec8<T>::load(buf, src + srow * (long)D + c8);
#pragma unroll
    for (int e = 0; e < 8; ++e)
      ScalarOps<T>::store(buf + e, s * ScalarOps<T>::load(buf + e));
    Vec8<T>::store(out + r * (long)D + c8, buf);
  }
}


template <typename T>
__global__ void rope_fwd_kernel(const T* __restrict__ x, const float* __restrict__ sin_t,
                                const float* __restrict__ cos_t, T* __restrict__ y,
                                long BH, int N, int P, int hd) {
  const int half = hd / 2;
  long total = BH * (long)N * half;
  for (long idx = blockIdx.x * (long)blockDim.x + threadIdx.x; idx < total;
       idx += (long)gridDim.x * blockDim.x) {
    int j = (int)(idx % half);
    long t = idx / half;
    int n = (int)(t % N);
    long base = t * (long)hd;
    int p = n - (N - P);
    float lo = ScalarOps<T>::load(x + base + j);
    float hi = ScalarOps<T>::load(x + base + half + j);
    if (p < 0) {
      ScalarOps<T>::store(y + base + j, lo);
      ScalarOps<T>::store(y + base + half + j, hi);
    } else {
      const float* srow = sin_t + (long)p * hd;
      const float* crow = cos_t + (long)p * hd;
      float s_lo = srow[j], c_lo = crow[j];
      float s_hi = srow[half + j], c_hi = crow[half + j];
      ScalarOps<T>::store(y + base + j, lo * c_lo - hi * s_lo);
      ScalarOps<T>::store(y + base + half + j, hi * c_hi + lo * s_hi);
    }
  }
}


template <typename T>
void launch_bias_gelu_fwd(const T* x, const T* bias, T* y, long rows, int H,
                          hipStream_t stream) {
  long total8 = rows * (long)(H / 8);
  int grid = (int)min((total8 + EW_BLOCK - 1) / EW_BLOCK, (long)2048);
  hipLaunchKernelGGL((bias_gelu_fwd_kernel<T>), dim3(grid), dim3(EW_BLOCK), 0, stream,
                     x, bias, y, rows, H);
}

template <typename T>
void launch_bias_gelu_bwd(const T* dy, const T* x, const T* bias, T* dx, float* dbias,
                          long rows, int H, hipStream_t stream) {
  const int col_tiles = (H / 8 + EW_BLOCK - 1) / EW_BLOCK;
  static const int rowsv = [] {
    const char* e = getenv("DINOV3_BG_ROWS");
    return e && e[0] == '1';
  }();
  if (rowsv && H == 4096) {
    int grid = (int)min(rows, (long)2048);
    hipLaunchKernelGGL((bias_gelu_bwd_rows_kernel<T, 2>), dim3(grid), dim3(256), 0,
                       stream, dy, x, bias, dx, dbias, rows, H);
    return;
  }
  static const int ilp8 = [] {
    const char* e = getenv("DINOV3_BG_ILP8");
    return e && e[0] == '1';
  }();
  if (ilp8) {
    int row_grid = (int)min((rows + 7) / 8, (long)(2048 / col_tiles + 1));
    hipLaunchKernelGGL((bias_gelu_bwd_kernel<T, 8>), dim3(row_grid, col_tiles),
                       dim3(EW_BLOCK), 0, stream, dy, x, bias, dx, dbias, rows, H);
    return;
  }
  int row_grid = (int)min((rows + 3) / 4, (long)(2048 / col_tiles + 1));
  hipLaunchKernelGGL((bias_gelu_bwd_kernel<T, 4>), dim3(row_grid, col_tiles),
                     dim3(EW_BLOCK), 0, stream, dy, x, bias, dx, dbias, rows, H);
}

template <typename T>
void launch_ls_axpy_fwd(const T* x, const T* res, const T* gamma, T* out, long rows,
                        int D, hipStream_t stream) {
  long total8 = rows * (long)(D / 8);
  int grid = (int)min((total8 + EW_BLOCK - 1) / EW_BLOCK, (long)2048);
  hipLaunchKernelGGL((ls_axpy_fwd_kernel<T>), dim3(grid), dim3(EW_BLOCK), 0, stream, x,
                     res, gamma, out, rows, D);
}

template <typename T>
void launch_ls_axpy_bwd(const T* dout, const T* res, const T* gamma, T* dres,
                        float* dgamma, long rows, int D, hipStream_t stream) {
  const int block = D / 8 < EW_BLOCK ? D / 8 : EW_BLOCK;
  const int col_tiles = (D / 8 + block - 1) / block;
  int row_grid = (int)min((rows + 7) / 8, (long)(1024 / col_tiles + 1));
  hipLaunchKernelGGL((ls_axpy_bwd_kernel<T>), dim3(row_grid, col_tiles), dim3(block),
                     0, stream, dout, res, gamma, dres, dgamma, rows, D);
}

template <typename T>
void launch_ls_axpy_bias_fwd(const T* x, const T* res, const T* gamma, const T* bias,
                             T* out, long rows, int D, hipStream_t stream) {
  long total8 = rows * (long)(D / 8);
  int grid = (int)min((total8 + EW_BLOCK - 1) / EW_BLOCK, (long)2048);
  hipLaunchKernelGGL((ls_axpy_bias_fwd_kernel<T>), dim3(grid), dim3(EW_BLOCK), 0, stream,
                     x, res, gamma, bias, out, rows, D);
}

template <typename T>
void launch_ls_axpy_bias_bwd(const T* dout, const T* res, const T* gamma, const T* bias,
                             T* dres, float* dgamma, float* dbias, long rows, int D,
                             hipStream_t stream) {
  const int block = D / 8 < EW_BLOCK ? D / 8 : EW_BLOCK;
  const int col_tiles = (D / 8 + block - 1) / block;
  int row_grid = (int)min((rows + 7) / 8, (long)(1024 / col_tiles + 1));
  hipLaunchKernelGGL((ls_axpy_bias_bwd_kernel<T>), dim3(row_grid, col_tiles),
                     dim3(block), 0, stream, dout, res, gamma, bias, dres, dgamma,
                     dbias, rows, D);
}

template <typename T>
void launch_ls_scatter_add(T* dst, const long* idx, const T* src, const T* gamma,
                           const T* bias, const float* scale, long M, int D,
                           hipStream_t stream) {
  long total = M * (long)(D / 8);
  int grid = (int)min((total + EW_BLOCK - 1) / EW_BLOCK, (long)2048);
  if (grid == 0) return;
  hipLaunchKernelGGL((ls_scatter_add_kernel<T>), dim3(grid), dim3(EW_BLOCK), 0, stream,
                     dst, idx, src, gamma, bias, scale, M, D);
}

template <typename T>
void launch_ls_scatter_bwd(const T* dy, const long* idx, const T* src, const T* gamma,
                           const T* bias, const float* scale, T* dres, float* dgamma,
                           float* dbias, long M, int D, hipStream_t stream) {
  const int block = D / 8 < EW_BLOCK ? D / 8 : EW_BLOCK;
  const int col_tiles = (D / 8 + block - 1) / block;
  int row_grid = (int)min(M > 0 ? (M + 7) / 8 : 1, (long)(1024 / col_tiles + 1));
  hipLaunchKernelGGL((ls_scatter_bwd_kernel<T, 4>), dim3(row_grid, col_tiles), dim3(block),
                     0, stream, dy, idx, src, gamma, bias, scale, dres, dgamma, dbias, M,
                     D);
}

template <typename T>
void launch_row_gather(const T* src, const long* idx, T* out, long M, int D,
                       hipStream_t stream) {
  long total = M * (long)(D / 8);
  int grid = (int)min((total + EW_BLOCK - 1) / EW_BLOCK, (long)2048);
  if (grid == 0) return;
  hipLaunchKernelGGL((row_gather_kernel<T>), dim3(grid), dim3(EW_BLOCK), 0, stream, src,
                     idx, out, M, D);
}

template <typename T>
void launch_row_scatter_add(T* dst, const long* idx, const T* src, const float* scale,
                            long M, int D, hipStream_t stream) {
  long total = M * (long)(D / 8);
  int grid = (int)min((total + EW_BLOCK - 1) / EW_BLOCK, (long)2048);
  if (grid == 0) return;
  hipLaunchKernelGGL((row_scatter_add_kernel<T>), dim3(grid), dim3(EW_BLOCK), 0, stream,
                     dst, idx, src, scale, M, D);
}

template <typename T>
void launch_row_gather_scaled(const T* src, const long* idx, const float* scale, T* out,
                              long M, int D, hipStream_t stream) {
  long total = M * (long)(D / 8);
  int grid = (int)min((total + EW_BLOCK - 1) / EW_BLOCK, (long)2048);
  if (grid == 0) return;
  hipLaunchKernelGGL((row_gather_scaled_kernel<T>), dim3(grid), dim3(EW_BLOCK), 0, stream,
                     src, idx, scale, out, M, D);
}

template <typename T>
void launch_swiglu_fwd(const T* x12, T* y, long rows, int H, hipStream_t stream) {
  long total = rows * (long)H;
  int grid = (int)min((total + EW_BLOCK - 1) / EW_BLOCK, (long)2048);
  hipLaunchKernelGGL((swiglu_fwd_kernel<T>), dim3(grid), dim3(EW_BLOCK), 0, stream,
                     x12, y, rows, H);
}

template <typename T>
void launch_swiglu_bwd(const T* dy, const T* x12, T* dx12, long rows, int H,
                       hipStream_t stream) {
  long total = rows * (long)H;
  int grid = (int)min((total + EW_BLOCK - 1) / EW_BLOCK, (long)2048);
  hipLaunchKernelGGL((swiglu_bwd_kernel<T>), dim3(grid), dim3(EW_BLOCK), 0, stream,
                     dy, x12, dx12, rows, H);
}

template <typename T>
void launch_rope_fwd(const T* x, const float* sin_t, const float* cos_t, T* y, long BH,
                     int N, int P, int hd, hipStream_t stream) {
  long total = BH * (long)N * (hd / 2);
  int grid = (int)min((total + EW_BLOCK - 1) / EW_BLOCK, (long)4096);
  hipLaunchKernelGGL((rope_fwd_kernel<T>), dim3(grid), dim3(EW_BLOCK), 0, stream,
                     x, sin_t, cos_t, y, BH, N, P, hd);
}

#define INSTANTIATE_EW(T)                                                            \
  template void launch_bias_gelu_fwd<T>(const T*, const T*, T*, long, int,           \
                                        hipStream_t);                                \
  template void launch_ls_axpy_fwd<T>(const T*, const T*, const T*, T*, long, int,   \
                                      hipStream_t);                                  \
  template void launch_ls_axpy_bwd<T>(const T*, const T*, const T*, T*, float*,      \
                                      long, int, hipStream_t);                       \
  template void launch_ls_axpy_bias_fwd<T>(const T*, const T*, const T*, const T*,   \
                                           T*, long, int, hipStream_t);              \
  template void launch_ls_axpy_bias_bwd<T>(const T*, const T*, const T*, const T*,   \
                                           T*, float*, float*, long, int,            \
                                           hipStream_t);                             \
  template void launch_ls_scatter_add<T>(T*, const long*, const T*, const T*,        \
                                         const T*, const float*, long, int,          \
                                         hipStream_t);                               \
  template void launch_ls_scatter_bwd<T>(const T*, const long*, const T*, const T*,  \
                                         const T*, const float*, T*, float*, float*, \
                                         long, int, hipStream_t);                    \
  template void launch_row_gather<T>(const T*, const long*, T*, long, int,           \
                                     hipStream_t);                                   \
  template void launch_row_scatter_add<T>(T*, const long*, const T*, const float*,   \
                                          long, int, hipStream_t);                   \
  template void launch_row_gather_scaled<T>(const T*, const long*, const float*, T*, \
                                            long, int, hipStream_t);                 \
  template void launch_bias_gelu_bwd<T>(const T*, const T*, const T*, T*, float*,    \
                                        long, int, hipStream_t);                     \
  template void launch_swiglu_fwd<T>(const T*, T*, long, int, hipStream_t);          \
  template void launch_swiglu_bwd<T>(const T*, const T*, T*, long, int, hipStream_t);\
  template void launch_rope_fwd<T>(const T*, const float*, const float*, T*, long,   \
                                   int, int, int, hipStream_t);

INSTANTIATE_EW(float)
INSTANTIATE_EW(__hip_bfloat16)
```

dinov3_amd/ops/csrc/norms.hip:

```cpp

#include "common.h"

#define LN_SHADOWS 32

#define NORM_BLOCK 256

static inline int norm_block_for(int D) {
  if (D >= 2048) return 256;
  if (D >= 1024) return 128;
  return 64;
}

template <typename T, bool V8>
DEV_INLINE void row_load8(const T* p, int i, float* out) {
  if constexpr (V8) {
    T buf[8];
    Vec8<T>::load(buf, p + i);
#pragma unroll
    for (int e = 0; e < 8; ++e) out[e] = ScalarOps<T>::load(buf + e);
  } else {
    out[0] = ScalarOps<T>::load(p + i);
  }
}

template <typename T, bool V8>
DEV_INLINE void row_store8(T* p, int i, const float* in) {
  if constexpr (V8) {
    T buf[8];
#pragma unroll
    for (int e = 0; e < 8; ++e) ScalarOps<T>::store(buf + e, in[e]);
    Vec8<T>::store(p + i, buf);
  } else {
    ScalarOps<T>::store(p + i, in[0]);
  }
}

#define ROW_LOOP(i) \
  for (int i = threadIdx.x * EW; i < D; i += blockDim.x * EW)


template <typename T, bool V8>
__global__ void layernorm_fwd_kernel(
    const T* __restrict__ x, const T* __restrict__ w, const T* __restrict__ b,
    T* __restrict__ y, float* __restrict__ mean_out, float* __restrict__ rstd_out,
    long rows, int D, float eps) {
  constexpr int EW = V8 ? 8 : 1;
  __shared__ float red[16];
  for (long row = blockIdx.x; row < rows; row += gridDim.x) {
    const T* xr = x + row * (long)D;
    T* yr = y + row * (long)D;
    float s = 0.f, s2 = 0.f;
    ROW_LOOP(i) {
      float v[EW];
      row_load8<T, V8>(xr, i, v);
#pragma unroll
      for (int e = 0; e < EW; ++e) {
        s += v[e];
        s2 += v[e] * v[e];
      }
    }
    s = block_reduce_sum(s, red);
    __syncthreads();
    s2 = block_reduce_sum(s2, red);
    float mean = s / D;
    float var = s2 / D - mean * mean;
    float rstd = rsqrtf(fmaxf(var, 0.f) + eps);
    if (threadIdx.x == 0) {
      mean_out[row] = mean;
      rstd_out[row] = rstd;
    }
    ROW_LOOP(i) {
      float v[EW], wv[EW], bv[EW], o[EW];
      row_load8<T, V8>(xr, i, v);
      row_load8<T, V8>(w, i, wv);
      row_load8<T, V8>(b, i, bv);
#pragma unroll
      for (int e = 0; e < EW; ++e) o[e] = (v[e] - mean) * rstd * wv[e] + bv[e];
      row_store8<T, V8>(yr, i, o);
    }
    __syncthreads();
  }
}

template <typename T, bool V8>
__global__ void layernorm_bwd_kernel(
    const T* __restrict__ dy, const T* __restrict__ x, const T* __restrict__ w,
    const float* __restrict__ mean, const float* __restrict__ rstd,
    T* __restrict__ dx, float* __restrict__ dw, float* __restrict__ db,
    long rows, int D) {
  constexpr int EW = V8 ? 8 : 1;
  extern __shared__ float smem[];
  float* red = smem;
  float* dw_acc = smem + 16;
  float* db_acc = dw_acc + D;
  for (int i = threadIdx.x; i < D; i += blockDim.x) {
    dw_acc[i] = 0.f;
    db_acc[i] = 0.f;
  }
  __syncthreads();
  for (long row = blockIdx.x; row < rows; row += gridDim.x) {
    const T* dyr = dy + row * (long)D;
    const T* xr = x + row * (long)D;
    T* dxr = dx + row * (long)D;
    const float m = mean[row], r = rstd[row];
    float sum_dyw = 0.f, sum_dyw_xhat = 0.f;
    ROW_LOOP(i) {
      float g[EW], v[EW], wv[EW];
      row_load8<T, V8>(dyr, i, g);
      row_load8<T, V8>(xr, i, v);
      row_load8<T, V8>(w, i, wv);
#pragma unroll
      for (int e = 0; e < EW; ++e) {
        const float xhat = (v[e] - m) * r;
        const float gw = g[e] * wv[e];
        sum_dyw += gw;
        sum_dyw_xhat += gw * xhat;
        dw_acc[i + e] += g[e] * xhat;
        db_acc[i + e] += g[e];
      }
    }
    sum_dyw = block_reduce_sum(sum_dyw, red);
    __syncthreads();
    sum_dyw_xhat = block_reduce_sum(sum_dyw_xhat, red);
    const float inv_d = 1.0f / D;
    ROW_LOOP(i) {
      float g[EW], v[EW], wv[EW], o[EW];
      row_load8<T, V8>(dyr, i, g);
      row_load8<T, V8>(xr, i, v);
      row_load8<T, V8>(w, i, wv);
#pragma unroll
      for (int e = 0; e < EW; ++e) {
        const float xhat = (v[e] - m) * r;
        o[e] = (g[e] * wv[e] - (sum_dyw + xhat * sum_dyw_xhat) * inv_d) * r;
      }
      row_store8<T, V8>(dxr, i, o);
    }
    __syncthreads();
  }
  float* dw_s = dw + (long)(blockIdx.x & (LN_SHADOWS - 1)) * D;
  float* db_s = db + (long)(blockIdx.x & (LN_SHADOWS - 1)) * D;
  for (int i = threadIdx.x; i < D; i += blockDim.x) {
    atomicAdd(dw_s + i, dw_acc[i]);
    atomicAdd(db_s + i, db_acc[i]);
  }
}

template <typename T, int CHUNKS>
__global__ __launch_bounds__(256) void layernorm_bwd_wave_kernel(
    const T* __restrict__ dy, const T* __restrict__ x, const T* __restrict__ w,
    const float* __restrict__ mean, const float* __restrict__ rstd,
    T* __restrict__ dx, float* __restrict__ dw, float* __restrict__ db,
    long rows, int D) {
  constexpr int NW = 4;
  const int wid = threadIdx.x / 64;
  const int lane = threadIdx.x & 63;
  extern __shared__ float smem[];
  float* dw_acc = smem + (long)wid * D;
  float* db_acc = smem + (long)(NW + wid) * D;
  for (int i = lane; i < D; i += 64) {
    dw_acc[i] = 0.f;
    db_acc[i] = 0.f;
  }
  float g[CHUNKS][8], v[CHUNKS][8], wv[CHUNKS][8];
  for (long row = (long)blockIdx.x * NW + wid; row < rows; row += (long)gridDim.x * NW) {
    const T* dyr = dy + row * (long)D;
    const T* xr = x + row * (long)D;
    const float m = mean[row], r = rstd[row];
    float sum_dyw = 0.f, sum_dyw_xhat = 0.f;
#pragma unroll
    for (int c = 0; c < CHUNKS; ++c) {
      const int i = (c * 64 + lane) * 8;
      if (i < D) {
        row_load8<T, true>(dyr, i, g[c]);
        row_load8<T, true>(xr, i, v[c]);
        row_load8<T, true>(w, i, wv[c]);
#pragma unroll
        for (int e = 0; e < 8; ++e) {
          const float xhat = (v[c][e] - m) * r;
          const float gw = g[c][e] * wv[c][e];
          sum_dyw += gw;
          sum_dyw_xhat += gw * xhat;
          dw_acc[i + e] += g[c][e] * xhat;
          db_acc[i + e] += g[c][e];
        }
      }
    }
#pragma unroll
    for (int off = 32; off > 0; off >>= 1) {
      sum_dyw += __shfl_xor(sum_dyw, off, 64);
      sum_dyw_xhat += __shfl_xor(sum_dyw_xhat, off, 64);
    }
    const float inv_d = 1.0f / D;
    T* dxr = dx + row * (long)D;
#pragma unroll
    for (int c = 0; c < CHUNKS; ++c) {
      const int i = (c * 64 + lane) * 8;
      if (i < D) {
        float o[8];
#pragma unroll
        for (int e = 0; e < 8; ++e) {
          const float xhat = (v[c][e] - m) * r;
          o[e] = (g[c][e] * wv[c][e] - (sum_dyw + xhat * sum_dyw_xhat) * inv_d) * r;
        }
        row_store8<T, true>(dxr, i, o);
      }
    }
  }
  __syncthreads();
  const long sh = (long)(blockIdx.x & (LN_SHADOWS - 1)) * D;
  for (int i = threadIdx.x; i < D; i += 256) {
    float a = 0.f, bsum = 0.f;
#pragma unroll
    for (int w2 = 0; w2 < NW; ++w2) {
      a += smem[(long)w2 * D + i];
      bsum += smem[(long)(NW + w2) * D + i];
    }
    atomicAdd(dw + sh + i, a);
    atomicAdd(db + sh + i, bsum);
  }
}


template <typename T, bool V8>
__global__ void rmsnorm_fwd_kernel(
    const T* __restrict__ x, const T* __restrict__ w, T* __restrict__ y,
    float* __restrict__ rstd_out, long rows, int D, float eps) {
  constexpr int EW = V8 ? 8 : 1;
  __shared__ float red[16];
  for (long row = blockIdx.x; row < rows; row += gridDim.x) {
    const T* xr = x + row * (long)D;
    T* yr = y + row * (long)D;
    float s2 = 0.f;
    ROW_LOOP(i) {
      float v[EW];
      row_load8<T, V8>(xr, i, v);
#pragma unroll
      for (int e = 0; e < EW; ++e) s2 += v[e] * v[e];
    }
    s2 = block_reduce_sum(s2, red);
    float rstd = rsqrtf(s2 / D + eps);
    if (threadIdx.x == 0) rstd_out[row] = rstd;
    ROW_LOOP(i) {
      float v[EW], wv[EW], o[EW];
      row_load8<T, V8>(xr, i, v);
      row_load8<T, V8>(w, i, wv);
#pragma unroll
      for (int e = 0; e < EW; ++e) o[e] = v[e] * rstd * wv[e];
      row_store8<T, V8>(yr, i, o);
    }
    __syncthreads();
  }
}

template <typename T, bool V8>
__global__ void rmsnorm_bwd_kernel(
    const T* __restrict__ dy, const T* __restrict__ x, const T* __restrict__ w,
    const float* __restrict__ rstd, T* __restrict__ dx, float* __restrict__ dw,
    long rows, int D) {
  constexpr int EW = V8 ? 8 : 1;
  extern __shared__ float smem[];
  float* red = smem;
  float* dw_acc = smem + 16;
  for (int i = threadIdx.x; i < D; i += blockDim.x) dw_acc[i] = 0.f;
  __syncthreads();
  for (long row = blockIdx.x; row < rows; row += gridDim.x) {
    const T* dyr = dy + row * (long)D;
    const T* xr = x + row * (long)D;
    T* dxr = dx + row * (long)D;
    const float r = rstd[row];
    float sum_gxw = 0.f;
    ROW_LOOP(i) {
      float g[EW], v[EW], wv[EW];
      row_load8<T, V8>(dyr, i, g);
      row_load8<T, V8>(xr, i, v);
      row_load8<T, V8>(w, i, wv);
#pragma unroll
      for (int e = 0; e < EW; ++e) {
        sum_gxw += g[e] * wv[e] * v[e];
        dw_acc[i + e] += g[e] * v[e] * r;
      }
    }
    sum_gxw = block_reduce_sum(sum_gxw, red);
    const float c = sum_gxw * r * r * r / D;
    ROW_LOOP(i) {
      float g[EW], v[EW], wv[EW], o[EW];
      row_load8<T, V8>(dyr, i, g);
      row_load8<T, V8>(xr, i, v);
      row_load8<T, V8>(w, i, wv);
#pragma unroll
      for (int e = 0; e < EW; ++e) o[e] = g[e] * wv[e] * r - v[e] * c;
      row_store8<T, V8>(dxr, i, o);
    }
    __syncthreads();
  }
  for (int i = threadIdx.x; i < D; i += blockDim.x) atomicAdd(dw + i, dw_acc[i]);
}


template <typename T, bool V8>
__global__ void l2norm_fwd_kernel(
    const T* __restrict__ x, T* __restrict__ y, float* __restrict__ s_out,
    long rows, int D, float eps) {
  constexpr int EW = V8 ? 8 : 1;
  __shared__ float red[16];
  for (long row = blockIdx.x; row < rows; row += gridDim.x) {
    const T* xr = x + row * (long)D;
    T* yr = y + row * (long)D;
    float s2 = 0.f;
    ROW_LOOP(i) {
      float v[EW];
      row_load8<T, V8>(xr, i, v);
#pragma unroll
      for (int e = 0; e < EW; ++e) s2 += v[e] * v[e];
    }
    s2 = block_reduce_sum(s2, red);
    float s = 1.0f / (sqrtf(s2) + eps);
    if (threadIdx.x == 0) s_out[row] = s;
    ROW_LOOP(i) {
      float v[EW], o[EW];
      row_load8<T, V8>(xr, i, v);
#pragma unroll
      for (int e = 0; e < EW; ++e) o[e] = v[e] * s;
      row_store8<T, V8>(yr, i, o);
    }
    __syncthreads();
  }
}

template <typename T, bool V8>
__global__ void l2norm_bwd_kernel(
    const T* __restrict__ dy, const T* __restrict__ y, const float* __restrict__ s_in,
    T* __restrict__ dx, long rows, int D, float eps) {
  constexpr int EW = V8 ? 8 : 1;
  __shared__ float red[16];
  for (long row = blockIdx.x; row < rows; row += gridDim.x) {
    const T* dyr = dy + row * (long)D;
    const T* yr = y + row * (long)D;
    T* dxr = dx + row * (long)D;
    const float s = s_in[row];
    const float n = 1.0f / s - eps;
    float dot = 0.f;
    ROW_LOOP(i) {
      float g[EW], v[EW];
      row_load8<T, V8>(dyr, i, g);
      row_load8<T, V8>(yr, i, v);
#pragma unroll
      for (int e = 0; e < EW; ++e) dot += g[e] * v[e];
    }
    dot = block_reduce_sum(dot, red);
    const float c = dot / fmaxf(n, 1e-20f);
    ROW_LOOP(i) {
      float g[EW], v[EW], o[EW];
      row_load8<T, V8>(dyr, i, g);
      row_load8<T, V8>(yr, i, v);
#pragma unroll
      for (int e = 0; e < EW; ++e) o[e] = s * g[e] - c * v[e];
      row_store8<T, V8>(dxr, i, o);
    }
    __syncthreads();
  }
}


#define DISPATCH_V8(D, ...)            \
  if ((D) % 8 == 0) {                  \
    constexpr bool V8 = true;          \
    __VA_ARGS__;                       \
  } else {                             \
    constexpr bool V8 = false;         \
    __VA_ARGS__;                       \
  }

template <typename T>
void launch_layernorm_fwd(const T* x, const T* w, const T* b, T* y, float* mean,
                          float* rstd, long rows, int D, float eps, hipStream_t stream) {
  int grid = (int)min(rows, (long)8192);
  DISPATCH_V8(D, hipLaunchKernelGGL(HIP_KERNEL_NAME(layernorm_fwd_kernel<T, V8>), dim3(grid),
                                     dim3(norm_block_for(D)), 0, stream, x, w, b, y, mean, rstd,
                                     rows, D, eps));
}

template <typename T>
void launch_layernorm_bwd(const T* dy, const T* x, const T* w, const float* mean,
                          const float* rstd, T* dx, float* dw, float* db, long rows,
                          int D, hipStream_t stream) {
  if (D % 8 == 0 && D <= 1536) {
    int grid = (int)min((rows + 3) / 4, (long)2048);
    size_t shmem = 2 * 4 * (size_t)D * sizeof(float);
    if (D <= 512)
      hipLaunchKernelGGL(HIP_KERNEL_NAME(layernorm_bwd_wave_kernel<T, 1>), dim3(grid),
                         dim3(256), shmem, stream, dy, x, w, mean, rstd, dx, dw, db,
                         rows, D);
    else if (D <= 1024)
      hipLaunchKernelGGL(HIP_KERNEL_NAME(layernorm_bwd_wave_kernel<T, 2>), dim3(grid),
                         dim3(256), shmem, stream, dy, x, w, mean, rstd, dx, dw, db,
                         rows, D);
    else
      hipLaunchKernelGGL(HIP_KERNEL_NAME(layernorm_bwd_wave_kernel<T, 3>), dim3(grid),
                         dim3(256), shmem, stream, dy, x, w, mean, rstd, dx, dw, db,
                         rows, D);
    return;
  }
  int grid = (int)min(rows, (long)2048);
  size_t shmem = (16 + 2 * (size_t)D) * sizeof(float);
  DISPATCH_V8(D, hipLaunchKernelGGL(HIP_KERNEL_NAME(layernorm_bwd_kernel<T, V8>), dim3(grid),
                                     dim3(norm_block_for(D)), shmem, stream, dy, x, w, mean,
                                     rstd, dx, dw, db, rows, D));
}

template <typename T>
void launch_rmsnorm_fwd(const T* x, const T* w, T* y, float* rstd, long rows, int D,
                        float eps, hipStream_t stream) {
  int grid = (int)min(rows, (long)8192);
  DISPATCH_V8(D, hipLaunchKernelGGL(HIP_KERNEL_NAME(rmsnorm_fwd_kernel<T, V8>), dim3(grid),
                                     dim3(norm_block_for(D)), 0, stream, x, w, y, rstd, rows, D,
                                     eps));
}

template <typename T>
void launch_rmsnorm_bwd(const T* dy, const T* x, const T* w, const float* rstd, T* dx,
                        float* dw, long rows, int D, hipStream_t stream) {
  int grid = (int)min(rows, (long)2048);
  size_t shmem = (16 + (size_t)D) * sizeof(float);
  DISPATCH_V8(D, hipLaunchKernelGGL(HIP_KERNEL_NAME(rmsnorm_bwd_kernel<T, V8>), dim3(grid),
                                     dim3(norm_block_for(D)), shmem, stream, dy, x, w, rstd, dx,
                                     dw, rows, D));
}

template <typename T>
void launch_l2norm_fwd(const T* x, T* y, float* s, long rows, int D, float eps,
                       hipStream_t stream) {
  int grid = (int)min(rows, (long)8192);
  DISPATCH_V8(D, hipLaunchKernelGGL(HIP_KERNEL_NAME(l2norm_fwd_kernel<T, V8>), dim3(grid),
                                     dim3(norm_block_for(D)), 0, stream, x, y, s, rows, D, eps));
}

template <typename T>
void launch_l2norm_bwd(const T* dy, const T* y, const float* s, T* dx, long rows, int D,
                       float eps, hipStream_t stream) {
  int grid = (int)min(rows, (long)8192);
  DISPATCH_V8(D, hipLaunchKernelGGL(HIP_KERNEL_NAME(l2norm_bwd_kernel<T, V8>), dim3(grid),
                                     dim3(norm_block_for(D)), 0, stream, dy, y, s, dx, rows, D,
                                     eps));
}

#define INSTANTIATE_NORMS(T)                                                              \
  template void launch_layernorm_fwd<T>(const T*, const T*, const T*, T*, float*, float*, \
                                        long, int, float, hipStream_t);                   \
  template void launch_layernorm_bwd<T>(const T*, const T*, const T*, const float*,       \
                                        const float*, T*, float*, float*, long, int,      \
                                        hipStream_t);                                     \
  template void launch_rmsnorm_fwd<T>(const T*, const T*, T*, float*, long, int, float,   \
                                      hipStream_t);                                       \
  template void launch_rmsnorm_bwd<T>(const T*, const T*, const T*, const float*, T*,     \
                                      float*, long, int, hipStream_t);                    \
  template void launch_l2norm_fwd<T>(const T*, T*, float*, long, int, float, hipStream_t);\
  template void launch_l2norm_bwd<T>(const T*, const T*, const float*, T*, long, int,     \
                                     float, hipStream_t);

INSTANTIATE_NORMS(float)
INSTANTIATE_NORMS(__hip_bfloat16)
```

Baseline: 478.7 images/sec.

## Replace atomic shadow column reductions with per-block partials and finalize kernel

Column-gradient reductions (dgamma, dbias, dw) in the norm and elementwise backward kernels now write one fp32 partial row per block into a workspace instead of using atomicAdd into 32 zeroed shadow rows. A dedicated finalize kernel sums the partials and writes the bf16 result, which removes the torch zeros/sum/cast ops on the host side. The GELU and bf16 packing were also rewritten with a sigmoid form and vector convert builtins, and layernorm bwd keeps its per-wave accumulators in registers. The change adds an extra kernel launch per op and a larger workspace, and grid sizes are now capped by the workspace rows.

```diff
diff --git a/dinov3_amd/ops/csrc/bindings.hip b/dinov3_amd/ops/csrc/bindings.hip
--- a/dinov3_amd/ops/csrc/bindings.hip
+++ b/dinov3_amd/ops/csrc/bindings.hip
@@ -6,6 +6,8 @@
 
 #include <vector>
 
+#include "common.h"
+
 #define CHECK_INPUT(x) \
   TORCH_CHECK(x.is_cuda() && x.is_contiguous(), #x " must be a contiguous HIP tensor")
 
@@ -14,36 +16,38 @@
                           float, hipStream_t);
 template <typename T>
 void launch_layernorm_bwd(const T*, const T*, const T*, const float*, const float*, T*,
-                          float*, float*, long, int, hipStream_t);
+                          float*, T*, T*, long, int, hipStream_t);
 template <typename T>
 void launch_rmsnorm_fwd(const T*, const T*, T*, float*, long, int, float, hipStream_t);
 template <typename T>
-void launch_rmsnorm_bwd(const T*, const T*, const T*, const float*, T*, float*, long, int,
+void launch_rmsnorm_bwd(const T*, const T*, const T*, const float*, T*, float*, T*, long,
+                        int, hipStream_t);
+template <typename T>
+void launch_l2norm_fwd(const T*, T*, float*, long, int, float, hipStream_t);
+template <typename T>
+void launch_l2norm_bwd(const T*, const T*, const float*, T*, long, int, float, hipStream_t);
+template <typename T>
+void launch_bias_gelu_fwd(const T*, const T*, T*, long, int, hipStream_t);
+template <typename T>
+void launch_bias_gelu_bwd(const T*, const T*, const T*, T*, float*, T*, long, int,
+                          hipStream_t);
+template <typename T>
+void launch_ls_axpy_fwd(const T*, const T*, const T*, T*, long, int, hipStream_t);
+template <typename T>
+void launch_ls_axpy_bwd(const T*, const T*, const T*, T*, float*, T*, long, int,
                         hipStream_t);
-template <typename T>
-void launch_l2norm_fwd(const T*, T*, float*, long, int, float, hipStream_t);
-template <typename T>
-void launch_l2norm_bwd(const T*, const T*, const float*, T*, long, int, float, hipStream_t);
-template <typename T>
-void launch_bias_gelu_fwd(const T*, const T*, T*, long, int, hipStream_t);
-template <typename T>
-void launch_bias_gelu_bwd(const T*, const T*, const T*, T*, float*, long, int, hipStream_t);
-template <typename T>
-void launch_ls_axpy_fwd(const T*, const T*, const T*, T*, long, int, hipStream_t);
-template <typename T>
-void launch_ls_axpy_bwd(const T*, const T*, const T*, T*, float*, long, int, hipStream_t);
 template <typename T>
 void launch_ls_axpy_bias_fwd(const T*, const T*, const T*, const T*, T*, long, int,
                              hipStream_t);
 template <typename T>
-void launch_ls_axpy_bias_bwd(const T*, const T*, const T*, const T*, T*, float*, float*,
+void launch_ls_axpy_bias_bwd(const T*, const T*, const T*, const T*, T*, float*, T*, T*,
                              long, int, hipStream_t);
 template <typename T>
 void launch_ls_scatter_add(T*, const long*, const T*, const T*, const T*, const float*,
                            long, int, hipStream_t);
 template <typename T>
 void launch_ls_scatter_bwd(const T*, const long*, const T*, const T*, const T*,
-                           const float*, T*, float*, float*, long, int, hipStream_t);
+                           const float*, T*, float*, T*, T*, long, int, hipStream_t);
 template <typename T>
 void launch_row_gather(const T*, const long*, T*, long, int, hipStream_t);
 template <typename T>
@@ -157,6 +161,11 @@
     }                                                                          \
   }()
 
+torch::Tensor colreduce_workspace(int n_acc, int D, const torch::Tensor& like) {
+  return torch::empty({(long)n_acc * COLRED_MAX_PARTIALS, D},
+                      like.options().dtype(torch::kFloat));
+}
+
 
 std::vector<torch::Tensor> layernorm_fwd(torch::Tensor x, torch::Tensor w, torch::Tensor b,
                                          double eps) {
@@ -183,16 +192,17 @@
   const int D = x.size(-1);
   const long rows = x.numel() / D;
   auto dx = torch::empty_like(x);
-  auto dw = torch::zeros({32, D}, x.options().dtype(torch::kFloat));
-  auto db = torch::zeros({32, D}, x.options().dtype(torch::kFloat));
+  auto dw = torch::empty({D}, x.options());
+  auto db = torch::empty({D}, x.options());
+  auto ws = colreduce_workspace(2, D, x);
   DISPATCH_FLOAT_BF16(x.scalar_type(), "layernorm_bwd", [&] {
     launch_layernorm_bwd<scalar_t>(
         (const scalar_t*)dy.data_ptr(), (const scalar_t*)x.data_ptr(),
         (const scalar_t*)w.data_ptr(), mean.data_ptr<float>(), rstd.data_ptr<float>(),
-        (scalar_t*)dx.data_ptr(), dw.data_ptr<float>(), db.data_ptr<float>(), rows, D,
-        current_stream());
-  });
-  return {dx, dw.sum(0).to(x.scalar_type()), db.sum(0).to(x.scalar_type())};
+        (scalar_t*)dx.data_ptr(), ws.data_ptr<float>(), (scalar_t*)dw.data_ptr(),
+        (scalar_t*)db.data_ptr(), rows, D, current_stream());
+  });
+  return {dx, dw, db};
 }
 
 std::vector<torch::Tensor> rmsnorm_fwd(torch::Tensor x, torch::Tensor w, double eps) {
@@ -215,14 +225,15 @@
   const int D = x.size(-1);
   const long rows = x.numel() / D;
   auto dx = torch::empty_like(x);
-  auto dw = torch::zeros({D}, x.options().dtype(torch::kFloat));
+  auto dw = torch::empty({D}, x.options());
+  auto ws = colreduce_workspace(1, D, x);
   DISPATCH_FLOAT_BF16(x.scalar_type(), "rmsnorm_bwd", [&] {
     launch_rmsnorm_bwd<scalar_t>((const scalar_t*)dy.data_ptr(), (const scalar_t*)x.data_ptr(),
                                  (const scalar_t*)w.data_ptr(), rstd.data_ptr<float>(),
-                                 (scalar_t*)dx.data_ptr(), dw.data_ptr<float>(), rows, D,
-                                 current_stream());
-  });
-  return {dx, dw.to(x.scalar_type())};
+                                 (scalar_t*)dx.data_ptr(), ws.data_ptr<float>(),
+                                 (scalar_t*)dw.data_ptr(), rows, D, current_stream());
+  });
+  return {dx, dw};
 }
 
 std::vector<torch::Tensor> l2norm_fwd(torch::Tensor x, double eps) {
@@ -272,14 +283,16 @@
   const int H = x.size(-1);
   const long rows = x.numel() / H;
   auto dx = torch::empty_like(x);
-  auto dbias = torch::zeros({32, H}, x.options().dtype(torch::kFloat));
+  auto dbias = torch::empty({H}, x.options());
+  auto ws = colreduce_workspace(1, H, x);
   DISPATCH_FLOAT_BF16(x.scalar_type(), "bias_gelu_bwd", [&] {
     launch_bias_gelu_bwd<scalar_t>((const scalar_t*)dy.data_ptr(),
                                    (const scalar_t*)x.data_ptr(),
                                    (const scalar_t*)bias.data_ptr(), (scalar_t*)dx.data_ptr(),
-                                   dbias.data_ptr<float>(), rows, H, current_stream());
-  });
-  return {dx, dbias.sum(0).to(x.scalar_type())};
+                                   ws.data_ptr<float>(), (scalar_t*)dbias.data_ptr(), rows, H,
+                                   current_stream());
+  });
+  return {dx, dbias};
 }
 
 torch::Tensor ls_axpy_fwd(torch::Tensor x, torch::Tensor res, torch::Tensor gamma) {
@@ -321,15 +334,16 @@
   const int D = dout.size(-1);
   const long rows = dout.numel() / D;
   auto dres = torch::empty_like(dout);
-  auto dgamma = torch::zeros({32, D}, dout.options().dtype(torch::kFloat));
+  auto dgamma = torch::empty({D}, dout.options());
+  auto ws = colreduce_workspace(1, D, dout);
   DISPATCH_FLOAT_BF16(dout.scalar_type(), "ls_axpy_bwd", [&] {
     launch_ls_axpy_bwd<scalar_t>((const scalar_t*)dout.data_ptr(),
                                  (const scalar_t*)res.data_ptr(),
                                  (const scalar_t*)gamma.data_ptr(),
-                                 (scalar_t*)dres.data_ptr(), dgamma.data_ptr<float>(),
-                                 rows, D, current_stream());
-  });
-  return {dres, dgamma.sum(0).to(dout.scalar_type())};
+                                 (scalar_t*)dres.data_ptr(), ws.data_ptr<float>(),
+                                 (scalar_t*)dgamma.data_ptr(), rows, D, current_stream());
+  });
+  return {dres, dgamma};
 }
 
 std::vector<torch::Tensor> ls_axpy_bias_bwd(torch::Tensor dout, torch::Tensor res,
@@ -338,17 +352,17 @@
   const int D = dout.size(-1);
   const long rows = dout.numel() / D;
   auto dres = torch::empty_like(dout);
-  auto fopt = dout.options().dtype(torch::kFloat);
-  auto dgamma = torch::zeros({32, D}, fopt);
-  auto dbias = torch::zeros({32, D}, fopt);
+  auto dgamma = torch::empty({D}, dout.options());
+  auto dbias = torch::empty({D}, dout.options());
+  auto ws = colreduce_workspace(2, D, dout);
   DISPATCH_FLOAT_BF16(dout.scalar_type(), "ls_axpy_bias_bwd", [&] {
     launch_ls_axpy_bias_bwd<scalar_t>(
         (const scalar_t*)dout.data_ptr(), (const scalar_t*)res.data_ptr(),
         (const scalar_t*)gamma.data_ptr(), (const scalar_t*)bias.data_ptr(),
-        (scalar_t*)dres.data_ptr(), dgamma.data_ptr<float>(), dbias.data_ptr<float>(),
-        rows, D, current_stream());
-  });
-  return {dres, dgamma.sum(0).to(dout.scalar_type()), dbias.sum(0).to(dout.scalar_type())};
+        (scalar_t*)dres.data_ptr(), ws.data_ptr<float>(), (scalar_t*)dgamma.data_ptr(),
+        (scalar_t*)dbias.data_ptr(), rows, D, current_stream());
+  });
+  return {dres, dgamma, dbias};
 }
 
 torch::Tensor row_gather(torch::Tensor src, torch::Tensor idx) {
@@ -417,9 +431,9 @@
   const int D = dy.size(-1);
   const long M = idx.numel();
   auto dres = torch::empty_like(src);
-  auto fopt = dy.options().dtype(torch::kFloat);
-  auto dgamma = gamma.defined() ? torch::zeros({32, D}, fopt) : torch::Tensor();
-  auto dbias = bias.defined() ? torch::zeros({32, D}, fopt) : torch::Tensor();
+  auto dgamma = gamma.defined() ? torch::empty({D}, dy.options()) : torch::Tensor();
+  auto dbias = bias.defined() ? torch::empty({D}, dy.options()) : torch::Tensor();
+  auto ws = colreduce_workspace(2, D, dy);
   DISPATCH_FLOAT_BF16(dy.scalar_type(), "ls_scatter_bwd", [&] {
     launch_ls_scatter_bwd<scalar_t>(
         (const scalar_t*)dy.data_ptr(), idx.data_ptr<long>(),
@@ -427,12 +441,11 @@
         gamma.defined() ? (const scalar_t*)gamma.data_ptr() : nullptr,
         bias.defined() ? (const scalar_t*)bias.data_ptr() : nullptr,
         scale.defined() && scale.numel() > 0 ? scale.data_ptr<float>() : nullptr,
-        (scalar_t*)dres.data_ptr(),
-        dgamma.defined() ? dgamma.data_ptr<float>() : nullptr,
-        dbias.defined() ? dbias.data_ptr<float>() : nullptr, M, D, current_stream());
-  });
-  return {dres, dgamma.defined() ? dgamma.sum(0).to(dy.scalar_type()) : dgamma,
-          dbias.defined() ? dbias.sum(0).to(dy.scalar_type()) : dbias};
+        (scalar_t*)dres.data_ptr(), ws.data_ptr<float>(),
+        dgamma.defined() ? (scalar_t*)dgamma.data_ptr() : nullptr,
+        dbias.defined() ? (scalar_t*)dbias.data_ptr() : nullptr, M, D, current_stream());
+  });
+  return {dres, dgamma, dbias};
 }
 
 torch::Tensor swiglu_fwd(torch::Tensor x12) {
diff --git a/dinov3_amd/ops/csrc/common.h b/dinov3_amd/ops/csrc/common.h
--- a/dinov3_amd/ops/csrc/common.h
+++ b/dinov3_amd/ops/csrc/common.h
@@ -9,6 +9,7 @@
 
 typedef __attribute__((ext_vector_type(8))) short short8_t;
 typedef __attribute__((ext_vector_type(4))) float float4_t;
+typedef __attribute__((ext_vector_type(4))) unsigned int uint4_t;
 
 DEV_INLINE float bf16_to_f32(short u) {
   union { float f; unsigned int i; } v;
@@ -16,12 +17,15 @@
   return v.f;
 }
 
-DEV_INLINE short f32_to_bf16(float f) {
-  union { float f; unsigned int i; } v;
-  v.f = f;
-  unsigned int rounding_bias = 0x7FFF + ((v.i >> 16) & 1);
-  return (short)((v.i + rounding_bias) >> 16);
+typedef __attribute__((ext_vector_type(2))) float float2_t;
+typedef __attribute__((ext_vector_type(2))) __bf16 bf16x2_t;
+
+DEV_INLINE unsigned int pack2_bf16(float lo, float hi) {
+  const float2_t f = {lo, hi};
+  return __builtin_bit_cast(unsigned int, __builtin_convertvector(f, bf16x2_t));
 }
+
+DEV_INLINE short f32_to_bf16(float f) { return (short)(pack2_bf16(f, 0.0f) & 0xFFFFu); }
 
 template <typename T> struct ScalarOps;
 
@@ -61,6 +65,26 @@
   }
   DEV_INLINE static void store(__hip_bfloat16* dst, const __hip_bfloat16* src) {
     *reinterpret_cast<float4_t*>(dst) = *reinterpret_cast<const float4_t*>(src);
+  }
+};
+
+template <typename T> struct Pack8 {
+  DEV_INLINE static void store(T* dst, const float* v) {
+    T buf[8];
+#pragma unroll
+    for (int e = 0; e < 8; ++e) ScalarOps<T>::store(buf + e, v[e]);
+    Vec8<T>::store(dst, buf);
+  }
+};
+
+template <> struct Pack8<__hip_bfloat16> {
+  DEV_INLINE static void store(__hip_bfloat16* dst, const float* v) {
+    uint4_t u;
+    u.x = pack2_bf16(v[0], v[1]);
+    u.y = pack2_bf16(v[2], v[3]);
+    u.z = pack2_bf16(v[4], v[5]);
+    u.w = pack2_bf16(v[6], v[7]);
+    *reinterpret_cast<uint4_t*>(dst) = u;
   }
 };
 
@@ -104,6 +128,57 @@
   return lds[0];
 }
 
+#define COLRED_MAX_PARTIALS 1024
+#define COLRED_COLS 64
+#define COLRED_SLICES 16
+
+static inline int even_row_grid(long groups, int cap) {
+  if (groups <= cap) return groups > 0 ? (int)groups : 1;
+  const long iters = (groups + cap - 1) / cap;
+  return (int)((groups + iters - 1) / iters);
+}
+
+template <typename T>
+__global__ __launch_bounds__(COLRED_COLS * COLRED_SLICES) void colreduce_finalize_kernel(
+    const float* __restrict__ part0, T* __restrict__ out0,
+    const float* __restrict__ part1, T* __restrict__ out1, int n_partials, int D) {
+  __shared__ float acc[COLRED_SLICES][COLRED_COLS];
+  const float* __restrict__ part = blockIdx.y == 0 ? part0 : part1;
+  T* __restrict__ out = blockIdx.y == 0 ? out0 : out1;
+  const int c = threadIdx.x & (COLRED_COLS - 1);
+  const int s = threadIdx.x / COLRED_COLS;
+  const int col = blockIdx.x * COLRED_COLS + c;
+  float sum = 0.f;
+  if (col < D) {
+#pragma unroll 8
+    for (int r = s; r < n_partials; r += COLRED_SLICES) sum += part[(long)r * D + col];
+  }
+  acc[s][c] = sum;
+  __syncthreads();
+  if (s == 0 && col < D) {
+    float t = acc[0][c];
+#pragma unroll
+    for (int k = 1; k < COLRED_SLICES; ++k) t += acc[k][c];
+    ScalarOps<T>::store(out + col, t);
+  }
+}
+
+template <typename T>
+static inline void launch_colreduce_finalize(const float* part0, T* out0, const float* part1,
+                                             T* out1, int n_partials, int D,
+                                             hipStream_t stream) {
+  if (part0 == nullptr) {
+    part0 = part1;
+    out0 = out1;
+    part1 = nullptr;
+  }
+  if (part0 == nullptr) return;
+  dim3 grid((D + COLRED_COLS - 1) / COLRED_COLS, part1 != nullptr ? 2 : 1);
+  hipLaunchKernelGGL(HIP_KERNEL_NAME(colreduce_finalize_kernel<T>), grid,
+                     dim3(COLRED_COLS * COLRED_SLICES), 0, stream, part0, out0, part1, out1,
+                     n_partials, D);
+}
+
 #define HIP_CHECK_LAUNCH()                                                    \
   do {                                                                        \
     hipError_t e = hipGetLastError();                                         \
diff --git a/dinov3_amd/ops/csrc/elementwise.hip b/dinov3_amd/ops/csrc/elementwise.hip
--- a/dinov3_amd/ops/csrc/elementwise.hip
+++ b/dinov3_amd/ops/csrc/elementwise.hip
@@ -2,138 +2,158 @@
 #include "common.h"
 
 #define EW_BLOCK 256
-#define EW_SHADOWS 32
-
-DEV_INLINE float fast_tanh(float y) {
-  return 1.0f - 2.0f / (1.0f + __expf(2.0f * y));
+#define EW_RED_BLOCK 512
+#define EW_RED_GRID 512
+#define EW_FWD_GRID 2048
+static_assert(EW_RED_GRID <= COLRED_MAX_PARTIALS, "workspace holds one row per block");
+
+DEV_INLINE float fast_sigmoid(float z) {
+  return __builtin_amdgcn_rcpf(1.0f + __expf(-z));
 }
 
 DEV_INLINE float gelu_tanh(float x) {
-  const float k0 = 0.7978845608028654f;
-  const float k1 = 0.044715f;
-  float inner = k0 * (x + k1 * x * x * x);
-  return 0.5f * x * (1.0f + fast_tanh(inner));
+  const float x2 = x * x;
+  return x * fast_sigmoid(x * (1.5957691216f + 0.07135481627f * x2));
 }
 
 DEV_INLINE float gelu_tanh_grad(float x) {
-  const float k0 = 0.7978845608028654f;
-  const float k1 = 0.044715f;
-  float x2 = x * x;
-  float inner = k0 * (x + k1 * x * x2);
-  float t = fast_tanh(inner);
-  float sech2 = 1.0f - t * t;
-  return 0.5f * (1.0f + t) + 0.5f * x * sech2 * k0 * (1.0f + 3.0f * k1 * x2);
-}
-
-
-template <typename T>
-__global__ void bias_gelu_fwd_kernel(const T* __restrict__ x, const T* __restrict__ bias,
-                                     T* __restrict__ y, long rows, int H) {
-  const long total8 = rows * (long)(H / 8);
-  for (long idx = blockIdx.x * (long)blockDim.x + threadIdx.x; idx < total8;
-       idx += (long)gridDim.x * blockDim.x) {
-    const int col8 = (int)(idx % (H / 8)) * 8;
-    const T* xp = x + idx * 8;
-    T* yp = y + idx * 8;
-    T xb[8], bb[8], yb[8];
-    Vec8<T>::load(xb, xp);
-    Vec8<T>::load(bb, bias + col8);
-#pragma unroll
-    for (int e = 0; e < 8; ++e) {
-      float v = ScalarOps<T>::load(xb + e) + ScalarOps<T>::load(bb + e);
-      ScalarOps<T>::store(yb + e, gelu_tanh(v));
-    }
-    Vec8<T>::store(yp, yb);
-  }
-}
-
-template <typename T, int RR_ILP = 4>
-__global__ void bias_gelu_bwd_kernel(const T* __restrict__ dy, const T* __restrict__ x,
-                                     const T* __restrict__ bias, T* __restrict__ dx,
-                                     float* __restrict__ dbias, long rows, int H) {
-  const int col8 = (blockIdx.y * blockDim.x + threadIdx.x) * 8;
-  if (col8 >= H) return;
-  T bb[8];
-  Vec8<T>::load(bb, bias + col8);
+  const float x2 = x * x;
+  const float s = fast_sigmoid(x * (1.5957691216f + 0.07135481627f * x2));
+  const float q = x * (1.5957691216f + 0.21406444881f * x2);
+  return s * (1.0f + q * (1.0f - s));
+}
+
+template <typename T>
+DEV_INLINE void load8_f32(const T* p, float* out) {
+  T buf[8];
+  Vec8<T>::load(buf, p);
+#pragma unroll
+  for (int e = 0; e < 8; ++e) out[e] = ScalarOps<T>::load(buf + e);
+}
+
+struct ColLane {
+  int col8;
+  int c;
+  int lr;
+  int rl;
+  bool active;
+};
+
+DEV_INLINE ColLane col_lane(int tpr, int D) {
+  ColLane t;
+  t.rl = blockDim.x / tpr;
+  t.lr = threadIdx.x / tpr;
+  t.c = threadIdx.x - t.lr * tpr;
+  t.col8 = (blockIdx.y * tpr + t.c) * 8;
+  t.active = t.lr < t.rl && t.col8 < D;
+  return t;
+}
+
+DEV_INLINE void colred_block_store(float* red, const float* acc, float* __restrict__ ws,
+                                   int D, int tpr, const ColLane& t) {
+  if (t.rl > 1) {
+    __syncthreads();
+    if (t.active && t.lr > 0) {
+      float4_t* r4 = reinterpret_cast<float4_t*>(red + threadIdx.x * 8);
+      r4[0] = float4_t{acc[0], acc[1], acc[2], acc[3]};
+      r4[1] = float4_t{acc[4], acc[5], acc[6], acc[7]};
+    }
+    __syncthreads();
+  }
+  if (t.active && t.lr == 0) {
+    float4_t lo = {acc[0], acc[1], acc[2], acc[3]};
+    float4_t hi = {acc[4], acc[5], acc[6], acc[7]};
+    for (int k = 1; k < t.rl; ++k) {
+      const float4_t* r4 = reinterpret_cast<const float4_t*>(red + (k * tpr + t.c) * 8);
+      lo += r4[0];
+      hi += r4[1];
+    }
+    float4_t* w4 = reinterpret_cast<float4_t*>(ws + (long)blockIdx.x * D + t.col8);
+    w4[0] = lo;
+    w4[1] = hi;
+  }
+}
+
+
+template <typename T, int RR = 4>
+__global__ __launch_bounds__(EW_BLOCK) void bias_gelu_fwd_kernel(
+    const T* __restrict__ x, const T* __restrict__ bias, T* __restrict__ y, long rows, int H,
+    int tpr) {
+  const ColLane t = col_lane(tpr, H);
+  if (!t.active) return;
+  float bb[8];
+  load8_f32(bias + t.col8, bb);
+  long row = ((long)blockIdx.x * t.rl + t.lr) * RR;
+  const long rstep = (long)gridDim.x * t.rl * RR;
+  for (; row + RR - 1 < rows; row += rstep) {
+    T xb[RR][8];
+#pragma unroll
+    for (int rr = 0; rr < RR; ++rr) Vec8<T>::load(xb[rr], x + (row + rr) * (long)H + t.col8);
+#pragma unroll
+    for (int rr = 0; rr < RR; ++rr) {
+      float o[8];
+#pragma unroll
+      for (int e = 0; e < 8; ++e) o[e] = gelu_tanh(ScalarOps<T>::load(xb[rr] + e) + bb[e]);
+      Pack8<T>::store(y + (row + rr) * (long)H + t.col8, o);
+    }
+  }
+  for (; row < rows; ++row) {
+    const long off = row * (long)H + t.col8;
+    float v[8], o[8];
+    load8_f32(x + off, v);
+#pragma unroll
+    for (int e = 0; e < 8; ++e) o[e] = gelu_tanh(v[e] + bb[e]);
+    Pack8<T>::store(y + off, o);
+  }
+}
+
+template <typename T, int RR = 4>
+__global__ __launch_bounds__(EW_RED_BLOCK, 4) void bias_gelu_bwd_kernel(
+    const T* __restrict__ dy, const T* __restrict__ x, const T* __restrict__ bias,
+    T* __restrict__ dx, float* __restrict__ dbias_ws, long rows, int H, int tpr) {
+  __shared__ float red[EW_RED_BLOCK * 8];
+  const ColLane t = col_lane(tpr, H);
   float db[8] = {0.f, 0.f, 0.f, 0.f, 0.f, 0.f, 0.f, 0.f};
-  long row = blockIdx.x * (long)RR_ILP;
-  const long rstep = (long)gridDim.x * RR_ILP;
-  for (; row + RR_ILP - 1 < rows; row += rstep) {
-    T xb[RR_ILP][8], gb[RR_ILP][8], ob[RR_ILP][8];
-#pragma unroll
-    for (int rr = 0; rr < RR_ILP; ++rr) {
-      const long off = (row + rr) * (long)H + col8;
-      Vec8<T>::load(xb[rr], x + off);
-      Vec8<T>::load(gb[rr], dy + off);
-    }
-#pragma unroll
-    for (int rr = 0; rr < RR_ILP; ++rr) {
+  if (t.active) {
+    float bb[8];
+    load8_f32(bias + t.col8, bb);
+    long row = ((long)blockIdx.x * t.rl + t.lr) * RR;
+    const long rstep = (long)gridDim.x * t.rl * RR;
+    for (; row + RR - 1 < rows; row += rstep) {
+      T xb[RR][8], gb[RR][8];
+#pragma unroll
+      for (int rr = 0; rr < RR; ++rr) {
+        const long off = (row + rr) * (long)H + t.col8;
+        Vec8<T>::load(xb[rr], x + off);
+        Vec8<T>::load(gb[rr], dy + off);
+      }
+      __builtin_amdgcn_sched_barrier(0);
+#pragma unroll
+      for (int rr = 0; rr < RR; ++rr) {
+        float o[8];
+#pragma unroll
+        for (int e = 0; e < 8; ++e) {
+          const float v = ScalarOps<T>::load(xb[rr] + e) + bb[e];
+          o[e] = ScalarOps<T>::load(gb[rr] + e) * gelu_tanh_grad(v);
+          db[e] += o[e];
+        }
+        Pack8<T>::store(dx + (row + rr) * (long)H + t.col8, o);
+      }
+    }
+    for (; row < rows; ++row) {
+      const long off = row * (long)H + t.col8;
+      float v[8], g[8], o[8];
+      load8_f32(x + off, v);
+      load8_f32(dy + off, g);
 #pragma unroll
       for (int e = 0; e < 8; ++e) {
-        float v = ScalarOps<T>::load(xb[rr] + e) + ScalarOps<T>::load(bb + e);
-        float g = ScalarOps<T>::load(gb[rr] + e) * gelu_tanh_grad(v);
-        ScalarOps<T>::store(ob[rr] + e, g);
-        db[e] += g;
+        o[e] = g[e] * gelu_tanh_grad(v[e] + bb[e]);
+        db[e] += o[e];
       }
-      Vec8<T>::store(dx + (row + rr) * (long)H + col8, ob[rr]);
-    }
-  }
-  for (; row < rows; ++row) {
-    const long off = row * (long)H + col8;
-    T xb[8], gb[8], ob[8];
-    Vec8<T>::load(xb, x + off);
-    Vec8<T>::load(gb, dy + off);
-#pragma unroll
-    for (int e = 0; e < 8; ++e) {
-      float v = ScalarOps<T>::load(xb + e) + ScalarOps<T>::load(bb + e);
-      float g = ScalarOps<T>::load(gb + e) * gelu_tanh_grad(v);
-      ScalarOps<T>::store(ob + e, g);
-      db[e] += g;
-    }
-    Vec8<T>::store(dx + off, ob);
-  }
-  float* dbias_s = dbias + (long)(blockIdx.x & (EW_SHADOWS - 1)) * H;
-#pragma unroll
-  for (int e = 0; e < 8; ++e) atomicAdd(dbias_s + col8 + e, db[e]);
-}
-
-template <typename T, int PASSES>
-__global__ __launch_bounds__(256) void bias_gelu_bwd_rows_kernel(
-    const T* __restrict__ dy, const T* __restrict__ x, const T* __restrict__ bias,
-    T* __restrict__ dx, float* __restrict__ dbias, long rows, int H) {
-  T bb[PASSES][8];
-  float db[PASSES][8];
-#pragma unroll
-  for (int pss = 0; pss < PASSES; ++pss) {
-    Vec8<T>::load(bb[pss], bias + (pss * 256 + threadIdx.x) * 8);
-#pragma unroll
-    for (int e = 0; e < 8; ++e) db[pss][e] = 0.f;
-  }
-  for (long row = blockIdx.x; row < rows; row += gridDim.x) {
-    const long base = row * (long)H;
-#pragma unroll
-    for (int pss = 0; pss < PASSES; ++pss) {
-      const long off = base + (pss * 256 + threadIdx.x) * 8;
-      T xb[8], gb[8], ob[8];
-      Vec8<T>::load(xb, x + off);
-      Vec8<T>::load(gb, dy + off);
-#pragma unroll
-      for (int e = 0; e < 8; ++e) {
-        const float v = ScalarOps<T>::load(xb + e) + ScalarOps<T>::load(bb[pss] + e);
-        const float g = ScalarOps<T>::load(gb + e) * gelu_tanh_grad(v);
-        ScalarOps<T>::store(ob + e, g);
-        db[pss][e] += g;
-      }
-      Vec8<T>::store(dx + off, ob);
-    }
-  }
-  float* dbias_s = dbias + (long)(blockIdx.x & (EW_SHADOWS - 1)) * H;
-#pragma unroll
-  for (int pss = 0; pss < PASSES; ++pss) {
-    const int c8 = (pss * 256 + threadIdx.x) * 8;
-#pragma unroll
-    for (int e = 0; e < 8; ++e) atomicAdd(dbias_s + c8 + e, db[pss][e]);
-  }
+      Pack8<T>::store(dx + off, o);
+    }
+  }
+  colred_block_store(red, db, dbias_ws, H, tpr, t);
 }
 
 
@@ -157,53 +177,6 @@
     }
     Vec8<T>::store(out + idx * 8, ob);
   }
-}
-
-template <typename T>
-__global__ void ls_axpy_bwd_kernel(const T* __restrict__ dout, const T* __restrict__ res,
-                                   const T* __restrict__ gamma, T* __restrict__ dres,
-                                   float* __restrict__ dgamma, long rows, int D) {
-  const int col8 = (blockIdx.y * blockDim.x + threadIdx.x) * 8;
-  if (col8 >= D) return;
-  T gb[8];
-  Vec8<T>::load(gb, gamma + col8);
-  float dg[8] = {0.f, 0.f, 0.f, 0.f, 0.f, 0.f, 0.f, 0.f};
-  long row = blockIdx.x * 4L;
-  const long rstep = (long)gridDim.x * 4;
-  for (; row + 3 < rows; row += rstep) {
-    T db[4][8], rb[4][8], ob[4][8];
-#pragma unroll
-    for (int rr = 0; rr < 4; ++rr) {
-      Vec8<T>::load(db[rr], dout + (row + rr) * (long)D + col8);
-      Vec8<T>::load(rb[rr], res + (row + rr) * (long)D + col8);
-    }
-#pragma unroll
-    for (int rr = 0; rr < 4; ++rr) {
-#pragma unroll
-      for (int e = 0; e < 8; ++e) {
-        const float g = ScalarOps<T>::load(db[rr] + e);
-        dg[e] += g * ScalarOps<T>::load(rb[rr] + e);
-        ScalarOps<T>::store(ob[rr] + e, g * ScalarOps<T>::load(gb + e));
-      }
-      Vec8<T>::store(dres + (row + rr) * (long)D + col8, ob[rr]);
-    }
-  }
-  for (; row < rows; ++row) {
-    const long off = row * (long)D + col8;
-    T db[8], rb[8], ob[8];
-    Vec8<T>::load(db, dout + off);
-    Vec8<T>::load(rb, res + off);
-#pragma unroll
-    for (int e = 0; e < 8; ++e) {
-      const float g = ScalarOps<T>::load(db + e);
-      dg[e] += g * ScalarOps<T>::load(rb + e);
-      ScalarOps<T>::store(ob + e, g * ScalarOps<T>::load(gb + e));
-    }
-    Vec8<T>::store(dres + off, ob);
-  }
-  float* dgamma_s = dgamma + (long)(blockIdx.x & (EW_SHADOWS - 1)) * D;
-#pragma unroll
-  for (int e = 0; e < 8; ++e) atomicAdd(dgamma_s + col8 + e, dg[e]);
 }
 
 
@@ -229,65 +202,6 @@
       ScalarOps<T>::store(ob + e, v);
     }
     Vec8<T>::store(out + idx * 8, ob);
-  }
-}
-
-template <typename T>
-__global__ void ls_axpy_bias_bwd_kernel(const T* __restrict__ dout,
-                                        const T* __restrict__ res,
-                                        const T* __restrict__ gamma,
-                                        const T* __restrict__ bias, T* __restrict__ dres,
-                                        float* __restrict__ dgamma,
-                                        float* __restrict__ dbias, long rows, int D) {
-  const int col8 = (blockIdx.y * blockDim.x + threadIdx.x) * 8;
-  if (col8 >= D) return;
-  T gb[8], bb[8];
-  Vec8<T>::load(gb, gamma + col8);
-  Vec8<T>::load(bb, bias + col8);
-  float dg[8] = {0.f, 0.f, 0.f, 0.f, 0.f, 0.f, 0.f, 0.f};
-  float db_acc[8] = {0.f, 0.f, 0.f, 0.f, 0.f, 0.f, 0.f, 0.f};
-  long row = blockIdx.x * 4L;
-  const long rstep = (long)gridDim.x * 4;
-  for (; row + 3 < rows; row += rstep) {
-    T db[4][8], rb[4][8], ob[4][8];
-#pragma unroll
-    for (int rr = 0; rr < 4; ++rr) {
-      Vec8<T>::load(db[rr], dout + (row + rr) * (long)D + col8);
-      Vec8<T>::load(rb[rr], res + (row + rr) * (long)D + col8);
-    }
-#pragma unroll
-    for (int rr = 0; rr < 4; ++rr) {
-#pragma unroll
-      for (int e = 0; e < 8; ++e) {
-        const float g = ScalarOps<T>::load(db[rr] + e);
-        const float gm = ScalarOps<T>::load(gb + e);
-        dg[e] += g * (ScalarOps<T>::load(rb[rr] + e) + ScalarOps<T>::load(bb + e));
-        db_acc[e] += g * gm;
-        ScalarOps<T>::store(ob[rr] + e, g * gm);
-      }
-      Vec8<T>::store(dres + (row + rr) * (long)D + col8, ob[rr]);
-    }
-  }
-  for (; row < rows; ++row) {
-    const long off = row * (long)D + col8;
-    T db[8], rb[8], ob[8];
-    Vec8<T>::load(db, dout + off);
-    Vec8<T>::load(rb, res + off);
-#pragma unroll
-    for (int e = 0; e < 8; ++e) {
-      const float g = ScalarOps<T>::load(db + e);
-      const float gm = ScalarOps<T>::load(gb + e);
-      dg[e] += g * (ScalarOps<T>::load(rb + e) + ScalarOps<T>::load(bb + e));
-      db_acc[e] += g * gm;
-      ScalarOps<T>::store(ob + e, g * gm);
-    }
-    Vec8<T>::store(dres + off, ob);
-  }
-  const long sh = (long)(blockIdx.x & (EW_SHADOWS - 1)) * D;
-#pragma unroll
-  for (int e = 0; e < 8; ++e) {
-    atomicAdd(dgamma + sh + col8 + e, dg[e]);
-    atomicAdd(dbias + sh + col8 + e, db_acc[e]);
   }
 }
 
@@ -322,71 +236,73 @@
   }
 }
 
-template <typename T, int RR = 4>
-__global__ void ls_scatter_bwd_kernel(const T* __restrict__ dy, const long* __restrict__ idx,
-                                      const T* __restrict__ src,
-                                      const T* __restrict__ gamma,
-                                      const T* __restrict__ bias,
-                                      const float* __restrict__ scale,
-                                      T* __restrict__ dres, float* __restrict__ dgamma,
-                                      float* __restrict__ dbias, long M, int D) {
-  const int col8 = (blockIdx.y * blockDim.x + threadIdx.x) * 8;
-  if (col8 >= D) return;
-  T gb[8], bb[8];
-  if (gamma != nullptr) Vec8<T>::load(gb, gamma + col8);
-  if (bias != nullptr) Vec8<T>::load(bb, bias + col8);
+template <typename T, bool INDEXED, int RR = 4>
+__global__ __launch_bounds__(EW_RED_BLOCK, 4) void ls_bwd_kernel(
+    const T* __restrict__ dy, const long* __restrict__ idx, const T* __restrict__ src,
+    const T* __restrict__ gamma, const T* __restrict__ bias, const float* __restrict__ scale,
+    T* __restrict__ dres, float* __restrict__ dgamma_ws, float* __restrict__ dbias_ws, long M,
+    int D, int tpr) {
+  __shared__ float red[EW_RED_BLOCK * 8];
+  const ColLane t = col_lane(tpr, D);
   float dg[8] = {0.f, 0.f, 0.f, 0.f, 0.f, 0.f, 0.f, 0.f};
-  float db_acc[8] = {0.f, 0.f, 0.f, 0.f, 0.f, 0.f, 0.f, 0.f};
-  long r = blockIdx.x * (long)RR;
-  const long rstep4 = (long)gridDim.x * RR;
-  for (; r + RR - 1 < M; r += rstep4) {
-    long srow[RR];
-    float sc[RR];
-    T dyb[RR][8], rb[RR][8], ob[RR][8];
-#pragma unroll
-    for (int rr = 0; rr < RR; ++rr) {
-      srow[rr] = idx[r + rr];
-      sc[rr] = scale != nullptr ? scale[r + rr] : 1.0f;
-      Vec8<T>::load(dyb[rr], dy + srow[rr] * (long)D + col8);
-      Vec8<T>::load(rb[rr], src + (r + rr) * (long)D + col8);
-    }
-#pragma unroll
-    for (int rr = 0; rr < RR; ++rr) {
+  float db[8] = {0.f, 0.f, 0.f, 0.f, 0.f, 0.f, 0.f, 0.f};
+  if (t.active) {
+    float gm[8], bv[8];
+#pragma unroll
+    for (int e = 0; e < 8; ++e) {
+      gm[e] = 1.0f;
+      bv[e] = 0.0f;
+    }
+    if (gamma != nullptr) load8_f32(gamma + t.col8, gm);
+    if (bias != nullptr) load8_f32(bias + t.col8, bv);
+    long r = ((long)blockIdx.x * t.rl + t.lr) * RR;
+    const long rstep = (long)gridDim.x * t.rl * RR;
+    for (; r + RR - 1 < M; r += rstep) {
+      long srow[RR];
+      float sc[RR];
+      T dyb[RR][8], rb[RR][8];
+#pragma unroll
+      for (int rr = 0; rr < RR; ++rr) {
+        srow[rr] = INDEXED ? idx[r + rr] : r + rr;
+        sc[rr] = scale != nullptr ? scale[r + rr] : 1.0f;
+      }
+#pragma unroll
+      for (int rr = 0; rr < RR; ++rr) {
+        Vec8<T>::load(dyb[rr], dy + srow[rr] * (long)D + t.col8);
+        Vec8<T>::load(rb[rr], src + (r + rr) * (long)D + t.col8);
+      }
+      __builtin_amdgcn_sched_barrier(0);
+#pragma unroll
+      for (int rr = 0; rr < RR; ++rr) {
+        float o[8];
+#pragma unroll
+        for (int e = 0; e < 8; ++e) {
+          const float gv = ScalarOps<T>::load(dyb[rr] + e) * sc[rr];
+          dg[e] += gv * (ScalarOps<T>::load(rb[rr] + e) + bv[e]);
+          o[e] = gv * gm[e];
+          db[e] += o[e];
+        }
+        Pack8<T>::store(dres + (r + rr) * (long)D + t.col8, o);
+      }
+    }
+    for (; r < M; ++r) {
+      const long srow = INDEXED ? idx[r] : r;
+      const float s = scale != nullptr ? scale[r] : 1.0f;
+      float g[8], v[8], o[8];
+      load8_f32(dy + srow * (long)D + t.col8, g);
+      load8_f32(src + r * (long)D + t.col8, v);
 #pragma unroll
       for (int e = 0; e < 8; ++e) {
-        const float gv = ScalarOps<T>::load(dyb[rr] + e) * sc[rr];
-        const float gm = gamma != nullptr ? ScalarOps<T>::load(gb + e) : 1.0f;
-        const float bv = bias != nullptr ? ScalarOps<T>::load(bb + e) : 0.0f;
-        dg[e] += gv * (ScalarOps<T>::load(rb[rr] + e) + bv);
-        db_acc[e] += gv * gm;
-        ScalarOps<T>::store(ob[rr] + e, gv * gm);
+        const float gv = g[e] * s;
+        dg[e] += gv * (v[e] + bv[e]);
+        o[e] = gv * gm[e];
+        db[e] += o[e];
       }
-      Vec8<T>::store(dres + (r + rr) * (long)D + col8, ob[rr]);
-    }
-  }
-  for (; r < M; ++r) {
-    const long srow = idx[r];
-    const float s = scale != nullptr ? scale[r] : 1.0f;
-    T dyb[8], rb[8], ob[8];
-    Vec8<T>::load(dyb, dy + srow * (long)D + col8);
-    Vec8<T>::load(rb, src + r * (long)D + col8);
-#pragma unroll
-    for (int e = 0; e < 8; ++e) {
-      const float gv = ScalarOps<T>::load(dyb + e) * s;
-      const float gm = gamma != nullptr ? ScalarOps<T>::load(gb + e) : 1.0f;
-      const float bv = bias != nullptr ? ScalarOps<T>::load(bb + e) : 0.0f;
-      dg[e] += gv * (ScalarOps<T>::load(rb + e) + bv);
-      db_acc[e] += gv * gm;
-      ScalarOps<T>::store(ob + e, gv * gm);
-    }
-    Vec8<T>::store(dres + r * (long)D + col8, ob);
-  }
-  const long sh = (long)(blockIdx.x & (EW_SHADOWS - 1)) * D;
-#pragma unroll
-  for (int e = 0; e < 8; ++e) {
-    if (dgamma != nullptr) atomicAdd(dgamma + sh + col8 + e, dg[e]);
-    if (dbias != nullptr) atomicAdd(dbias + sh + col8 + e, db_acc[e]);
-  }
+      Pack8<T>::store(dres + r * (long)D + t.col8, o);
+    }
+  }
+  if (dgamma_ws != nullptr) colred_block_store(red, dg, dgamma_ws, D, tpr, t);
+  if (dbias_ws != nullptr) colred_block_store(red, db, dbias_ws, D, tpr, t);
 }
 
 
@@ -401,7 +317,7 @@
     const T* xr = x12 + row * (long)(2 * H);
     float x1 = ScalarOps<T>::load(xr + col);
     float x2 = ScalarOps<T>::load(xr + H + col);
-    float sig = 1.0f / (1.0f + expf(-x1));
+    float sig = __builtin_amdgcn_rcpf(1.0f + expf(-x1));
     ScalarOps<T>::store(y + idx, x1 * sig * x2);
   }
 }
@@ -419,7 +335,7 @@
     float x1 = ScalarOps<T>::load(xr + col);
     float x2 = ScalarOps<T>::load(xr + H + col);
     float g = ScalarOps<T>::load(dy + idx);
-    float sig = 1.0f / (1.0f + expf(-x1));
+    float sig = __builtin_amdgcn_rcpf(1.0f + expf(-x1));
     float silu = x1 * sig;
     float dsilu = sig * (1.0f + x1 * (1.0f - sig));
     ScalarOps<T>::store(dxr + col, g * x2 * dsilu);
@@ -521,42 +437,54 @@
 }
 
 
+struct ColGrid {
+  int tpr, col_tiles, row_grid;
+};
+
+static ColGrid col_grid(long rows, int D, int block, int max_blocks, int rr) {
+  ColGrid g;
+  const int d8 = D / 8;
+  g.tpr = d8 < block ? d8 : block;
+  g.col_tiles = (d8 + g.tpr - 1) / g.tpr;
+  const long rows_per_iter = (long)(block / g.tpr) * rr;
+  const int cap = max_blocks / g.col_tiles > 0 ? max_blocks / g.col_tiles : 1;
+  g.row_grid = even_row_grid((rows + rows_per_iter - 1) / rows_per_iter, cap);
+  return g;
+}
+
 template <typename T>
 void launch_bias_gelu_fwd(const T* x, const T* bias, T* y, long rows, int H,
                           hipStream_t stream) {
-  long total8 = rows * (long)(H / 8);
-  int grid = (int)min((total8 + EW_BLOCK - 1) / EW_BLOCK, (long)2048);
-  hipLaunchKernelGGL((bias_gelu_fwd_kernel<T>), dim3(grid), dim3(EW_BLOCK), 0, stream,
-                     x, bias, y, rows, H);
-}
-
-template <typename T>
-void launch_bias_gelu_bwd(const T* dy, const T* x, const T* bias, T* dx, float* dbias,
-                          long rows, int H, hipStream_t stream) {
-  const int col_tiles = (H / 8 + EW_BLOCK - 1) / EW_BLOCK;
-  static const int rowsv = [] {
-    const char* e = getenv("DINOV3_BG_ROWS");
-    return e && e[0] == '1';
-  }();
-  if (rowsv && H == 4096) {
-    int grid = (int)min(rows, (long)2048);
-    hipLaunchKernelGGL((bias_gelu_bwd_rows_kernel<T, 2>), dim3(grid), dim3(256), 0,
-                       stream, dy, x, bias, dx, dbias, rows, H);
-    return;
-  }
-  static const int ilp8 = [] {
-    const char* e = getenv("DINOV3_BG_ILP8");
-    return e && e[0] == '1';
-  }();
-  if (ilp8) {
-    int row_grid = (int)min((rows + 7) / 8, (long)(2048 / col_tiles + 1));
-    hipLaunchKernelGGL((bias_gelu_bwd_kernel<T, 8>), dim3(row_grid, col_tiles),
-                       dim3(EW_BLOCK), 0, stream, dy, x, bias, dx, dbias, rows, H);
-    return;
-  }
-  int row_grid = (int)min((rows + 3) / 4, (long)(2048 / col_tiles + 1));
-  hipLaunchKernelGGL((bias_gelu_bwd_kernel<T, 4>), dim3(row_grid, col_tiles),
-                     dim3(EW_BLOCK), 0, stream, dy, x, bias, dx, dbias, rows, H);
+  const ColGrid g = col_grid(rows, H, EW_BLOCK, EW_FWD_GRID, 4);
+  hipLaunchKernelGGL((bias_gelu_fwd_kernel<T, 4>), dim3(g.row_grid, g.col_tiles),
+                     dim3(EW_BLOCK), 0, stream, x, bias, y, rows, H, g.tpr);
+}
+
+template <typename T>
+void launch_bias_gelu_bwd(const T* dy, const T* x, const T* bias, T* dx, float* ws,
+                          T* dbias, long rows, int H, hipStream_t stream) {
+  const ColGrid g = col_grid(rows, H, EW_RED_BLOCK, EW_RED_GRID, 4);
+  hipLaunchKernelGGL((bias_gelu_bwd_kernel<T, 4>), dim3(g.row_grid, g.col_tiles),
+                     dim3(EW_RED_BLOCK), 0, stream, dy, x, bias, dx, ws, rows, H, g.tpr);
+  launch_colreduce_finalize<T>(ws, dbias, nullptr, nullptr, g.row_grid, H, stream);
+}
+
+template <typename T>
+static void launch_ls_bwd(const T* dy, const long* idx, const T* src, const T* gamma,
+                          const T* bias, const float* scale, T* dres, float* ws, T* dgamma,
+                          T* dbias, long M, int D, hipStream_t stream) {
+  const ColGrid g = col_grid(M, D, EW_RED_BLOCK, EW_RED_GRID, 4);
+  float* ws_g = dgamma != nullptr ? ws : nullptr;
+  float* ws_b = dbias != nullptr ? ws + (long)COLRED_MAX_PARTIALS * D : nullptr;
+  if (idx != nullptr)
+    hipLaunchKernelGGL((ls_bwd_kernel<T, true, 4>), dim3(g.row_grid, g.col_tiles),
+                       dim3(EW_RED_BLOCK), 0, stream, dy, idx, src, gamma, bias, scale, dres,
+                       ws_g, ws_b, M, D, g.tpr);
+  else
+    hipLaunchKernelGGL((ls_bwd_kernel<T, false, 4>), dim3(g.row_grid, g.col_tiles),
+                       dim3(EW_RED_BLOCK), 0, stream, dy, idx, src, gamma, bias, scale, dres,
+                       ws_g, ws_b, M, D, g.tpr);
+  launch_colreduce_finalize<T>(ws_g, dgamma, ws_b, dbias, g.row_grid, D, stream);
 }
 
 template <typename T>
@@ -569,13 +497,10 @@
 }
 
 template <typename T>
-void launch_ls_axpy_bwd(const T* dout, const T* res, const T* gamma, T* dres,
-                        float* dgamma, long rows, int D, hipStream_t stream) {
-  const int block = D / 8 < EW_BLOCK ? D / 8 : EW_BLOCK;
-  const int col_tiles = (D / 8 + block - 1) / block;
-  int row_grid = (int)min((rows + 7) / 8, (long)(1024 / col_tiles + 1));
-  hipLaunchKernelGGL((ls_axpy_bwd_kernel<T>), dim3(row_grid, col_tiles), dim3(block),
-                     0, stream, dout, res, gamma, dres, dgamma, rows, D);
+void launch_ls_axpy_bwd(const T* dout, const T* res, const T* gamma, T* dres, float* ws,
+                        T* dgamma, long rows, int D, hipStream_t stream) {
+  launch_ls_bwd<T>(dout, nullptr, res, gamma, nullptr, nullptr, dres, ws, dgamma, nullptr,
+                   rows, D, stream);
 }
 
 template <typename T>
@@ -589,14 +514,10 @@
 
 template <typename T>
 void launch_ls_axpy_bias_bwd(const T* dout, const T* res, const T* gamma, const T* bias,
-                             T* dres, float* dgamma, float* dbias, long rows, int D,
+                             T* dres, float* ws, T* dgamma, T* dbias, long rows, int D,
                              hipStream_t stream) {
-  const int block = D / 8 < EW_BLOCK ? D / 8 : EW_BLOCK;
-  const int col_tiles = (D / 8 + block - 1) / block;
-  int row_grid = (int)min((rows + 7) / 8, (long)(1024 / col_tiles + 1));
-  hipLaunchKernelGGL((ls_axpy_bias_bwd_kernel<T>), dim3(row_grid, col_tiles),
-                     dim3(block), 0, stream, dout, res, gamma, bias, dres, dgamma,
-                     dbias, rows, D);
+  launch_ls_bwd<T>(dout, nullptr, res, gamma, bias, nullptr, dres, ws, dgamma, dbias, rows,
+                   D, stream);
 }
 
 template <typename T>
@@ -612,14 +533,9 @@
 
 template <typename T>
 void launch_ls_scatter_bwd(const T* dy, const long* idx, const T* src, const T* gamma,
-                           const T* bias, const float* scale, T* dres, float* dgamma,
-                           float* dbias, long M, int D, hipStream_t stream) {
-  const int block = D / 8 < EW_BLOCK ? D / 8 : EW_BLOCK;
-  const int col_tiles = (D / 8 + block - 1) / block;
-  int row_grid = (int)min(M > 0 ? (M + 7) / 8 : 1, (long)(1024 / col_tiles + 1));
-  hipLaunchKernelGGL((ls_scatter_bwd_kernel<T, 4>), dim3(row_grid, col_tiles), dim3(block),
-                     0, stream, dy, idx, src, gamma, bias, scale, dres, dgamma, dbias, M,
-                     D);
+                           const T* bias, const float* scale, T* dres, float* ws, T* dgamma,
+                           T* dbias, long M, int D, hipStream_t stream) {
+  launch_ls_bwd<T>(dy, idx, src, gamma, bias, scale, dres, ws, dgamma, dbias, M, D, stream);
 }
 
 template <typename T>
@@ -683,18 +599,18 @@
                                         hipStream_t);                                \
   template void launch_ls_axpy_fwd<T>(const T*, const T*, const T*, T*, long, int,   \
                                       hipStream_t);                                  \
-  template void launch_ls_axpy_bwd<T>(const T*, const T*, const T*, T*, float*,      \
+  template void launch_ls_axpy_bwd<T>(const T*, const T*, const T*, T*, float*, T*,  \
                                       long, int, hipStream_t);                       \
   template void launch_ls_axpy_bias_fwd<T>(const T*, const T*, const T*, const T*,   \
                                            T*, long, int, hipStream_t);              \
   template void launch_ls_axpy_bias_bwd<T>(const T*, const T*, const T*, const T*,   \
-                                           T*, float*, float*, long, int,            \
+                                           T*, float*, T*, T*, long, int,            \
                                            hipStream_t);                             \
   template void launch_ls_scatter_add<T>(T*, const long*, const T*, const T*,        \
                                          const T*, const float*, long, int,          \
                                          hipStream_t);                               \
   template void launch_ls_scatter_bwd<T>(const T*, const long*, const T*, const T*,  \
-                                         const T*, const float*, T*, float*, float*, \
+                                         const T*, const float*, T*, float*, T*, T*, \
                                          long, int, hipStream_t);                    \
   template void launch_row_gather<T>(const T*, const long*, T*, long, int,           \
                                      hipStream_t);                                   \
@@ -703,7 +619,7 @@
   template void launch_row_gather_scaled<T>(const T*, const long*, const float*, T*, \
                                             long, int, hipStream_t);                 \
   template void launch_bias_gelu_bwd<T>(const T*, const T*, const T*, T*, float*,    \
-                                        long, int, hipStream_t);                     \
+                                        T*, long, int, hipStream_t);                 \
   template void launch_swiglu_fwd<T>(const T*, T*, long, int, hipStream_t);          \
   template void launch_swiglu_bwd<T>(const T*, const T*, T*, long, int, hipStream_t);\
   template void launch_rope_fwd<T>(const T*, const float*, const float*, T*, long,   \
diff --git a/dinov3_amd/ops/csrc/norms.hip b/dinov3_amd/ops/csrc/norms.hip
--- a/dinov3_amd/ops/csrc/norms.hip
+++ b/dinov3_amd/ops/csrc/norms.hip
@@ -1,9 +1,9 @@
 
 #include "common.h"
 
-#define LN_SHADOWS 32
-
 #define NORM_BLOCK 256
+#define LN_BWD_GRID 1024
+static_assert(LN_BWD_GRID <= COLRED_MAX_PARTIALS, "workspace holds one row per block");
 
 static inline int norm_block_for(int D) {
   if (D >= 2048) return 256;
@@ -26,10 +26,7 @@
 template <typename T, bool V8>
 DEV_INLINE void row_store8(T* p, int i, const float* in) {
   if constexpr (V8) {
-    T buf[8];
-#pragma unroll
-    for (int e = 0; e < 8; ++e) ScalarOps<T>::store(buf + e, in[e]);
-    Vec8<T>::store(p + i, buf);
+    Pack8<T>::store(p + i, in);
   } else {
     ScalarOps<T>::store(p + i, in[0]);
   }
@@ -86,7 +83,7 @@
 __global__ void layernorm_bwd_kernel(
     const T* __restrict__ dy, const T* __restrict__ x, const T* __restrict__ w,
     const float* __restrict__ mean, const float* __restrict__ rstd,
-    T* __restrict__ dx, float* __restrict__ dw, float* __restrict__ db,
+    T* __restrict__ dx, float* __restrict__ dw_ws, float* __restrict__ db_ws,
     long rows, int D) {
   constexpr int EW = V8 ? 8 : 1;
   extern __shared__ float smem[];
@@ -137,11 +134,11 @@
     }
     __syncthreads();
   }
-  float* dw_s = dw + (long)(blockIdx.x & (LN_SHADOWS - 1)) * D;
-  float* db_s = db + (long)(blockIdx.x & (LN_SHADOWS - 1)) * D;
+  float* dw_row = dw_ws + (long)blockIdx.x * D;
+  float* db_row = db_ws + (long)blockIdx.x * D;
   for (int i = threadIdx.x; i < D; i += blockDim.x) {
-    atomicAdd(dw_s + i, dw_acc[i]);
-    atomicAdd(db_s + i, db_acc[i]);
+    dw_row[i] = dw_acc[i];
+    db_row[i] = db_acc[i];
   }
 }
 
@@ -149,39 +146,51 @@
 __global__ __launch_bounds__(256) void layernorm_bwd_wave_kernel(
     const T* __restrict__ dy, const T* __restrict__ x, const T* __restrict__ w,
     const float* __restrict__ mean, const float* __restrict__ rstd,
-    T* __restrict__ dx, float* __restrict__ dw, float* __restrict__ db,
+    T* __restrict__ dx, float* __restrict__ dw_ws, float* __restrict__ db_ws,
     long rows, int D) {
   constexpr int NW = 4;
   const int wid = threadIdx.x / 64;
   const int lane = threadIdx.x & 63;
   extern __shared__ float smem[];
-  float* dw_acc = smem + (long)wid * D;
-  float* db_acc = smem + (long)(NW + wid) * D;
-  for (int i = lane; i < D; i += 64) {
-    dw_acc[i] = 0.f;
-    db_acc[i] = 0.f;
-  }
-  float g[CHUNKS][8], v[CHUNKS][8], wv[CHUNKS][8];
+  float wv[CHUNKS][8], dw_acc[CHUNKS][8], db_acc[CHUNKS][8];
+#pragma unroll
+  for (int c = 0; c < CHUNKS; ++c) {
+    const int i = (c * 64 + lane) * 8;
+#pragma unroll
+    for (int e = 0; e < 8; ++e) {
+      wv[c][e] = 0.f;
+      dw_acc[c][e] = 0.f;
+      db_acc[c][e] = 0.f;
+    }
+    if (i < D) row_load8<T, true>(w, i, wv[c]);
+  }
+  const float inv_d = 1.0f / D;
   for (long row = (long)blockIdx.x * NW + wid; row < rows; row += (long)gridDim.x * NW) {
     const T* dyr = dy + row * (long)D;
     const T* xr = x + row * (long)D;
     const float m = mean[row], r = rstd[row];
-    float sum_dyw = 0.f, sum_dyw_xhat = 0.f;
+    float g[CHUNKS][8], xhat[CHUNKS][8];
 #pragma unroll
     for (int c = 0; c < CHUNKS; ++c) {
       const int i = (c * 64 + lane) * 8;
       if (i < D) {
         row_load8<T, true>(dyr, i, g[c]);
-        row_load8<T, true>(xr, i, v[c]);
-        row_load8<T, true>(w, i, wv[c]);
+        row_load8<T, true>(xr, i, xhat[c]);
+      }
+    }
+    float sum_dyw = 0.f, sum_dyw_xhat = 0.f;
+#pragma unroll
+    for (int c = 0; c < CHUNKS; ++c) {
+      const int i = (c * 64 + lane) * 8;
+      if (i < D) {
 #pragma unroll
         for (int e = 0; e < 8; ++e) {
-          const float xhat = (v[c][e] - m) * r;
+          xhat[c][e] = (xhat[c][e] - m) * r;
           const float gw = g[c][e] * wv[c][e];
           sum_dyw += gw;
-          sum_dyw_xhat += gw * xhat;
-          dw_acc[i + e] += g[c][e] * xhat;
-          db_acc[i + e] += g[c][e];
+          sum_dyw_xhat += gw * xhat[c][e];
+          dw_acc[c][e] += g[c][e] * xhat[c][e];
+          db_acc[c][e] += g[c][e];
         }
       }
     }
@@ -190,7 +199,6 @@
       sum_dyw += __shfl_xor(sum_dyw, off, 64);
       sum_dyw_xhat += __shfl_xor(sum_dyw_xhat, off, 64);
     }
-    const float inv_d = 1.0f / D;
     T* dxr = dx + row * (long)D;
 #pragma unroll
     for (int c = 0; c < CHUNKS; ++c) {
@@ -198,25 +206,34 @@
       if (i < D) {
         float o[8];
 #pragma unroll
-        for (int e = 0; e < 8; ++e) {
-          const float xhat = (v[c][e] - m) * r;
-          o[e] = (g[c][e] * wv[c][e] - (sum_dyw + xhat * sum_dyw_xhat) * inv_d) * r;
-        }
+        for (int e = 0; e < 8; ++e)
+          o[e] = (g[c][e] * wv[c][e] - (sum_dyw + xhat[c][e] * sum_dyw_xhat) * inv_d) * r;
         row_store8<T, true>(dxr, i, o);
       }
     }
   }
-  __syncthreads();
-  const long sh = (long)(blockIdx.x & (LN_SHADOWS - 1)) * D;
-  for (int i = threadIdx.x; i < D; i += 256) {
-    float a = 0.f, bsum = 0.f;
-#pragma unroll
-    for (int w2 = 0; w2 < NW; ++w2) {
-      a += smem[(long)w2 * D + i];
-      bsum += smem[(long)(NW + w2) * D + i];
-    }
-    atomicAdd(dw + sh + i, a);
-    atomicAdd(db + sh + i, bsum);
+#pragma unroll
+  for (int pass = 0; pass < 2; ++pass) {
+    if (pass == 1) __syncthreads();
+#pragma unroll
+    for (int c = 0; c < CHUNKS; ++c) {
+      const int i = (c * 64 + lane) * 8;
+      if (i < D) {
+        const float* a = pass == 0 ? dw_acc[c] : db_acc[c];
+        float4_t* s4 = reinterpret_cast<float4_t*>(smem + (long)wid * D + i);
+        s4[0] = float4_t{a[0], a[1], a[2], a[3]};
+        s4[1] = float4_t{a[4], a[5], a[6], a[7]};
+      }
+    }
+    __syncthreads();
+    float* out_row = (pass == 0 ? dw_ws : db_ws) + (long)blockIdx.x * D;
+    for (int i = threadIdx.x * 4; i < D; i += 256 * 4) {
+      float4_t a = *reinterpret_cast<const float4_t*>(smem + i);
+#pragma unroll
+      for (int w2 = 1; w2 < NW; ++w2)
+        a += *reinterpret_cast<const float4_t*>(smem + (long)w2 * D + i);
+      *reinterpret_cast<float4_t*>(out_row + i) = a;
+    }
   }
 }
 
@@ -255,7 +272,7 @@
 template <typename T, bool V8>
 __global__ void rmsnorm_bwd_kernel(
     const T* __restrict__ dy, const T* __restrict__ x, const T* __restrict__ w,
-    const float* __restrict__ rstd, T* __restrict__ dx, float* __restrict__ dw,
+    const float* __restrict__ rstd, T* __restrict__ dx, float* __restrict__ dw_ws,
     long rows, int D) {
   constexpr int EW = V8 ? 8 : 1;
   extern __shared__ float smem[];
@@ -293,7 +310,8 @@
     }
     __syncthreads();
   }
-  for (int i = threadIdx.x; i < D; i += blockDim.x) atomicAdd(dw + i, dw_acc[i]);
+  float* dw_row = dw_ws + (long)blockIdx.x * D;
+  for (int i = threadIdx.x; i < D; i += blockDim.x) dw_row[i] = dw_acc[i];
 }
 
 
@@ -382,30 +400,34 @@
 
 template <typename T>
 void launch_layernorm_bwd(const T* dy, const T* x, const T* w, const float* mean,
-                          const float* rstd, T* dx, float* dw, float* db, long rows,
+                          const float* rstd, T* dx, float* ws, T* dw, T* db, long rows,
                           int D, hipStream_t stream) {
+  float* dw_ws = ws;
+  float* db_ws = ws + (long)COLRED_MAX_PARTIALS * D;
+  int grid;
   if (D % 8 == 0 && D <= 1536) {
-    int grid = (int)min((rows + 3) / 4, (long)2048);
-    size_t shmem = 2 * 4 * (size_t)D * sizeof(float);
+    grid = even_row_grid((rows + 3) / 4, D <= 1024 ? LN_BWD_GRID : LN_BWD_GRID * 3 / 4);
+    size_t shmem = 4 * (size_t)D * sizeof(float);
     if (D <= 512)
       hipLaunchKernelGGL(HIP_KERNEL_NAME(layernorm_bwd_wave_kernel<T, 1>), dim3(grid),
-                         dim3(256), shmem, stream, dy, x, w, mean, rstd, dx, dw, db,
+                         dim3(256), shmem, stream, dy, x, w, mean, rstd, dx, dw_ws, db_ws,
                          rows, D);
     else if (D <= 1024)
       hipLaunchKernelGGL(HIP_KERNEL_NAME(layernorm_bwd_wave_kernel<T, 2>), dim3(grid),
-                         dim3(256), shmem, stream, dy, x, w, mean, rstd, dx, dw, db,
+                         dim3(256), shmem, stream, dy, x, w, mean, rstd, dx, dw_ws, db_ws,
                          rows, D);
     else
       hipLaunchKernelGGL(HIP_KERNEL_NAME(layernorm_bwd_wave_kernel<T, 3>), dim3(grid),
-                         dim3(256), shmem, stream, dy, x, w, mean, rstd, dx, dw, db,
+                         dim3(256), shmem, stream, dy, x, w, mean, rstd, dx, dw_ws, db_ws,
                          rows, D);
-    return;
-  }
-  int grid = (int)min(rows, (long)2048);
-  size_t shmem = (16 + 2 * (size_t)D) * sizeof(float);
-  DISPATCH_V8(D, hipLaunchKernelGGL(HIP_KERNEL_NAME(layernorm_bwd_kernel<T, V8>), dim3(grid),
-                                     dim3(norm_block_for(D)), shmem, stream, dy, x, w, mean,
-                                     rstd, dx, dw, db, rows, D));
+  } else {
+    grid = even_row_grid(rows, LN_BWD_GRID);
+    size_t shmem = (16 + 2 * (size_t)D) * sizeof(float);
+    DISPATCH_V8(D, hipLaunchKernelGGL(HIP_KERNEL_NAME(layernorm_bwd_kernel<T, V8>), dim3(grid),
+                                       dim3(norm_block_for(D)), shmem, stream, dy, x, w, mean,
+                                       rstd, dx, dw_ws, db_ws, rows, D));
+  }
+  launch_colreduce_finalize<T>(dw_ws, dw, db_ws, db, grid, D, stream);
 }
 
 template <typename T>
@@ -419,12 +441,13 @@
 
 template <typename T>
 void launch_rmsnorm_bwd(const T* dy, const T* x, const T* w, const float* rstd, T* dx,
-                        float* dw, long rows, int D, hipStream_t stream) {
-  int grid = (int)min(rows, (long)2048);
+                        float* ws, T* dw, long rows, int D, hipStream_t stream) {
+  int grid = even_row_grid(rows, LN_BWD_GRID);
   size_t shmem = (16 + (size_t)D) * sizeof(float);
   DISPATCH_V8(D, hipLaunchKernelGGL(HIP_KERNEL_NAME(rmsnorm_bwd_kernel<T, V8>), dim3(grid),
                                      dim3(norm_block_for(D)), shmem, stream, dy, x, w, rstd, dx,
-                                     dw, rows, D));
+                                     ws, rows, D));
+  launch_colreduce_finalize<T>(ws, dw, nullptr, nullptr, grid, D, stream);
 }
 
 template <typename T>
@@ -448,12 +471,12 @@
   template void launch_layernorm_fwd<T>(const T*, const T*, const T*, T*, float*, float*, \
                                         long, int, float, hipStream_t);                   \
   template void launch_layernorm_bwd<T>(const T*, const T*, const T*, const float*,       \
-                                        const float*, T*, float*, float*, long, int,      \
+                                        const float*, T*, float*, T*, T*, long, int,      \
                                         hipStream_t);                                     \
   template void launch_rmsnorm_fwd<T>(const T*, const T*, T*, float*, long, int, float,   \
                                       hipStream_t);                                       \
   template void launch_rmsnorm_bwd<T>(const T*, const T*, const T*, const float*, T*,     \
-                                      float*, long, int, hipStream_t);                    \
+                                      float*, T*, long, int, hipStream_t);                \
   template void launch_l2norm_fwd<T>(const T*, T*, float*, long, int, float, hipStream_t);\
   template void launch_l2norm_bwd<T>(const T*, const T*, const float*, T*, long, int,     \
                                      float, hipStream_t);
```

After: 518.2 images/sec (median of 6 runs). 1.08x the previous value.
